# Isomorpfishm/SINGA

Hardware: AMD Instinct MI355X
Metric: protein-ligand graphs/sec GAN step (G+D fwd+bwd); scatter-TP kernel HBM GB/s (higher is better)
Workload: dtype f32

## Files before the change

### singa_amd/csrc/singa_hip.hip

```cpp
#include <hip/hip_runtime.h>
#include <hip/hip_ext.h>

#include <math.h>
#include <stdint.h>
#include <stdio.h>
#include <string.h>
#include <type_traits>

#include "../../include/singa_hip.h"
#include "../../include/singa_hip_lab.h"
#include "../../include/singa_hip_gen.h"
#include "../../include/singa_hip_force.h"
#include "so3_index.h"

namespace {

thread_local char g_err[256] = "ok";

int fail(int code, const char* msg) {
    snprintf(g_err, sizeof(g_err), "%s", msg);
    return code;
}

int check_launch(const char* what) {
// ... 3207 lines not shown
    const int n0 = (int)(blockIdx.x / HV) * npb;
    const int n1 = n0 + npb < N ? n0 + npb : N;
    if (n0 >= n1) return;
    float w[L + 1][4][4];
#pragma unroll
    for (int l = 0; l <= L; ++l)
#pragma unroll
        for (int t = 0; t < 4; ++t)
#pragma unroll
            for (int j = 0; j < 4; ++j) w[l][t][j] = W[l * w_l + (cc + t) * w_c + (4 * g + j) * w_u];
    float4 bc = make_float4(0.f, 0.f, 0.f, 0.f);
    if (bias) bc = *reinterpret_cast<const float4*>(bias + cc);
    for (int nb = n0; nb < n1; nb += 16) {
        const int na = nb + i < n1 ? nb + i : n1 - 1;
        const float* arow = small + (long long)na * K * 16 + 4 * g;
        float4 a = *reinterpret_cast<const float4*>(arow);
#pragma unroll
        for (int k = 0; k < K; ++k) {
            float4 an = a;
            if (k + 1 < K) an = *reinterpret_cast<const float4*>(arow + (k + 1) * 16);
            int l = 0;
            while ((l + 1) * (l + 1) <= k) ++l;
            const float av[4] = {a.x, a.y, a.z, a.w};
            floatx4 acc[4];
#pragma unroll
            for (int t = 0; t < 4; ++t) {
                const float b0 = k == 0 ? (t == 0 ? bc.x : (t == 1 ? bc.y : (t == 2 ? bc.z : bc.w))) : 0.f;
                acc[t] = floatx4{b0, b0, b0, b0};
            }
#pragma unroll
            for (int j = 0; j < 4; ++j)
#pragma unroll
                for (int t = 0; t < 4; ++t) acc[t] = __builtin_amdgcn_mfma_f32_16x16x4f32(av[j], w[l][t][j], acc[t], 0, 0, 0);
#pragma unroll
            for (int r = 0; r < 4; ++r) {
                const int n = nb + 4 * g + r;
                if (act && n < n1)
                    *reinterpret_cast<float4*>(big + ((long long)n * K + k) * C + cc) = make_float4(acc[0][r], acc[1][r], acc[2][r], acc[3][r]);
            }
            a = an;
        }
    }
}

template <int L>
struct SkinnyChunk {
    static constexpr int K = (L + 1) * (L + 1);
    static constexpr int D = L == 2 ? 3 : (L == 4 ? 5 : 7);
};

template <int L, int C>
__global__ void __launch_bounds__(SkinnyCfg<C>::BLOCK) so3_skinny_reduce_mfma_kernel(const float* __restrict__ small, const float* __restrict__ big,
                                                                     float* __restrict__ part, int N, int npb, int out_cu,
                                                                     int bias_row) {
    constexpr int K = (L + 1) * (L + 1), HV = SkinnyCfg<C>::HALVES, BL = SkinnyCfg<C>::BLOCK, D = SkinnyChunk<L>::D, NCH = K / D;
    static_assert(NCH * D == K, "chunking");
    const int lane = threadIdx.x & 63, i = lane & 15, g = lane >> 4;
    const int c0 = ((int)(blockIdx.x % HV) * (BL / 64) + (int)(threadIdx.x >> 6)) * 64 + 4 * i;
    const bool act = c0 + 3 < C;
    const int cc = act ? c0 : C - 4;
    const int n0 = (int)(blockIdx.x / HV) * npb;
    const int n1 = n0 + npb < N ? n0 + npb : N;
    floatx4 acc[L + 1][4];
#pragma unroll
    for (int l = 0; l <= L; ++l)
#pragma unroll
        for (int t = 0; t < 4; ++t) acc[l][t] = floatx4{0.f, 0.f, 0.f, 0.f};
    float4 accb = make_float4(0.f, 0.f, 0.f, 0.f);
    if (n0 < n1) {
        float4 bcur[D], bnxt[D];
        float acur[D], anxt[D];
        auto load = [&](float4* b, float* a, int q, int ch) {
            const int n = q + g;
            const bool ok = n < n1;
            const long long nn = ok ? n : n1 - 1;
#pragma unroll
            for (int d = 0; d < D; ++d) {
                const int k = ch * D + d;
                b[d] = *reinterpret_cast<const float4*>(big + (nn * K + k) * C + cc);
                const float v = small[(nn * K + k) * 16 + i];
                a[d] = ok ? v : 0.f;
            }
        };
        load(bnxt, anxt, n0, 0);
        for (int q = n0; q < n1; q += 4) {
#pragma unroll
            for (int ch = 0; ch < NCH; ++ch) {
#pragma unroll
                for (int d = 0; d < D; ++d) bcur[d] = bnxt[d], acur[d] = anxt[d];
                if (ch + 1 < NCH) load(bnxt, anxt, q, ch + 1);
                else load(bnxt, anxt, q + 4 < n1 ? q + 4 : q, 0);
#pragma unroll
                for (int d = 0; d < D; ++d) {
                    const int k = ch * D + d;
                    int l = 0;
                    while ((l + 1) * (l + 1) <= k) ++l;
                    const float bv[4] = {bcur[d].x, bcur[d].y, bcur[d].z, bcur[d].w};
#pragma unroll
                    for (int t = 0; t < 4; ++t) acc[l][t] = __builtin_amdgcn_mfma_f32_16x16x4f32(acur[d], bv[t], acc[l][t], 0, 0, 0);
                    if (k == 0 && q + g < n1) {
                        accb.x += bv[0]; accb.y += bv[1]; accb.z += bv[2]; accb.w += bv[3];
                    }
                }
            }
        }
    }
    constexpr int WSZ_ = (L + 1) * 16 * C;
    float* p = part + (long long)(blockIdx.x / HV) * (WSZ_ + (bias_row ? C : 0));
    if (bias_row) {
        accb.x += __shfl_xor(accb.x, 16, 64); accb.y += __shfl_xor(accb.y, 16, 64); accb.z += __shfl_xor(accb.z, 16, 64); accb.w += __shfl_xor(accb.w, 16, 64);
        accb.x += __shfl_xor(accb.x, 32, 64); accb.y += __shfl_xor(accb.y, 32, 64); accb.z += __shfl_xor(accb.z, 32, 64); accb.w += __shfl_xor(accb.w, 32, 64);
    }
    if (!act) return;
#pragma unroll
    for (int l = 0; l <= L; ++l) {
        if (out_cu) {
#pragma unroll
            for (int t = 0; t < 4; ++t)
                *reinterpret_cast<float4*>(p + ((long long)l * C + cc + t) * 16 + 4 * g) = make_float4(acc[l][t][0], acc[l][t][1], acc[l][t][2], acc[l][t][3]);
        } else {
#pragma unroll
            for (int r = 0; r < 4; ++r)
                *reinterpret_cast<float4*>(p + ((long long)l * 16 + 4 * g + r) * C + cc) = make_float4(acc[l][0][r], acc[l][1][r], acc[l][2][r], acc[l][3][r]);
        }
    }
    if (bias_row && g == 0) *reinterpret_cast<float4*>(p + WSZ_ + cc) = accb;
}

static inline int so3_skinny_npb(int N, int target_blocks) {
    int npb = (N + target_blocks - 1) / target_blocks;
    return npb < 8 ? 8 : npb;
}

template <int C>
static int so3_skinny_reduce_runs(int lmax) {
    static int cached[8] = {0};
    if (lmax < 0 || lmax > 7) return 512;
    if (cached[lmax]) return cached[lmax];
    int per_cu = 0, cus = 256;
    hipError_t e = hipErrorInvalidValue;
    constexpr int BL = SkinnyCfg<C>::BLOCK;
    if (lmax == 2) e = hipOccupancyMaxActiveBlocksPerMultiprocessor(&per_cu, so3_skinny_reduce_kernel<2, C>, BL, 0);
    if (lmax == 4) e = hipOccupancyMaxActiveBlocksPerMultiprocessor(&per_cu, so3_skinny_reduce_kernel<4, C>, BL, 0);
    if (lmax == 6) e = hipOccupancyMaxActiveBlocksPerMultiprocessor(&per_cu, so3_skinny_reduce_kernel<6, C>, BL, 0);
    if (e != hipSuccess || per_cu < 1) per_cu = 2;
    int dev = 0;
    hipDeviceProp_t prop;
    if (hipGetDevice(&dev) == hipSuccess && hipGetDeviceProperties(&prop, dev) == hipSuccess && prop.multiProcessorCount > 0)
        cus = prop.multiProcessorCount;
    cached[lmax] = per_cu * cus / SkinnyCfg<C>::HALVES;
    return cached[lmax];
}
static inline bool so3_skinny_channels_ok(int C) { return C == 512 || C == 112; }

__device__ __forceinline__ float group16_sum(float v) {
    v += __shfl_xor(v, 1, 64);
    v += __shfl_xor(v, 2, 64);
    v += __shfl_xor(v, 4, 64);
    v += __shfl_xor(v, 8, 64);
    return v;
}
__host__ __device__ constexpr int deg_of_c(int k) {
    int l = 0;
    while ((l + 1) * (l + 1) <= k) ++l;
    return l;
}
__host__ __device__ constexpr float bal_of_c(int k, int L) { return 1.0f / (float)((2 * deg_of_c(k) + 1) * (L + 1)); }

template <int L>
__global__ void __launch_bounds__(64) rmsnorm_fwd4_kernel(const float* __restrict__ x, const float* __restrict__ weight,
                                                          const float* __restrict__ bias, float* __restrict__ y, int N, float eps) {
    constexpr int C = 16, K = (L + 1) * (L + 1), KC = K * C;
    const int lane = threadIdx.x, q = lane >> 4, c = lane & 15;
    float w[L + 1];
#pragma unroll
    for (int l = 0; l <= L; ++l) w[l] = weight[l * C + c];
    const float bc = bias[c];
    for (int n0 = 4 * (int)blockIdx.x; n0 < N; n0 += 4 * (int)gridDim.x) {
        const int n = n0 + q;
        const bool ok = n < N;
        const float* xi = x + (long long)(ok ? n : N - 1) * KC + c;
        float v[K];
#pragma clang loop unroll(full)
        for (int k = 0; k < K; ++k) v[k] = xi[k * C];
        v[0] -= group16_sum(v[0]) * (1.0f / C);
        float ss = 0.f;
#pragma clang loop unroll(full)
        for (int k = 0; k < K; ++k) ss = fmaf(v[k] * v[k], bal_of_c(k, L), ss);
        const float r = rsqrtf(group16_sum(ss) * (1.0f / C) + eps);
        if (ok) {
            float* yo = y + (long long)n * KC + c;
#pragma clang loop unroll(full)
            for (int k = 0; k < K; ++k) {
                const float rw = r * w[deg_of_c(k)];
                yo[k * C] = k == 0 ? fmaf(v[k], rw, bc) : v[k] * rw;
            }
        }
    }
}

template <int L, bool ADD>
__global__ void __launch_bounds__(64) rmsnorm_bwd4_kernel(const float* __restrict__ x, const float* __restrict__ weight,
                                                          const float* __restrict__ gy, const float* __restrict__ g_add,
                                                          float* __restrict__ gx, float* __restrict__ gw_part,
                                                          float* __restrict__ gb_part, int N, float eps) {
    constexpr int C = 16, K = (L + 1) * (L + 1), KC = K * C;
    const int lane = threadIdx.x, q = lane >> 4, c = lane & 15;
    float w[L + 1], gwp[L + 1];
#pragma unroll
    for (int l = 0; l <= L; ++l) { w[l] = weight[l * C + c]; gwp[l] = 0.f; }
    float gbp = 0.f;
    for (int n0 = 4 * (int)blockIdx.x; n0 < N; n0 += 4 * (int)gridDim.x) {
        const int n = n0 + q;
        const bool ok = n < N;
        const long long base = (long long)(ok ? n : N - 1) * KC + c;
        float v[K], g[K], ga[ADD ? K : 1];
#pragma clang loop unroll(full)
        for (int k = 0; k < K; ++k) {
            v[k] = x[base + k * C];
            g[k] = gy[base + k * C];
            if constexpr (ADD) ga[k] = g_add[base + k * C];
        }
        const float live = ok ? 1.f : 0.f;
        v[0] -= group16_sum(v[0]) * (1.0f / C);
        float ss = 0.f, gl[L + 1];
#pragma unroll
        for (int l = 0; l <= L; ++l) gl[l] = 0.f;
#pragma clang loop unroll(full)
        for (int k = 0; k < K; ++k) {
            ss = fmaf(v[k] * v[k], bal_of_c(k, L), ss);
            gl[deg_of_c(k)] = fmaf(g[k], v[k], gl[deg_of_c(k)]);
        }
        float S = 0.f;
#pragma unroll
        for (int l = 0; l <= L; ++l) S = fmaf(gl[l], w[l], S);
        gbp = fmaf(g[0], live, gbp);
        const float r = rsqrtf(group16_sum(ss) * (1.0f / C) + eps);
        S = group16_sum(S);
        const float r3s = r * r * r * S * (1.0f / C);
#pragma unroll
        for (int l = 0; l <= L; ++l) gwp[l] = fmaf(gl[l] * live, r, gwp[l]);
        float* go = gx + base;
        float d0 = fmaf(r * w[0], g[0], -r3s * bal_of_c(0, L) * v[0]);
        d0 -= group16_sum(d0) * (1.0f / C);
        if (ok) {
            go[0] = ADD ? d0 + ga[0] : d0;
#pragma clang loop unroll(full)
            for (int k = 1; k < K; ++k) {
                const float d = fmaf(r * w[deg_of_c(k)], g[k], -r3s * bal_of_c(k, L) * v[k]);
                go[k * C] = ADD ? d + ga[k] : d;
            }
        }
    }
#pragma unroll
    for (int l = 0; l <= L; ++l) {
        gwp[l] += __shfl_xor(gwp[l], 16, 64);
        gwp[l] += __shfl_xor(gwp[l], 32, 64);
    }
    gbp += __shfl_xor(gbp, 16, 64);
    gbp += __shfl_xor(gbp, 32, 64);
    if (lane < C) {
        float* wp = gw_part + (long long)blockIdx.x * (L + 1) * C;
#pragma unroll
        for (int l = 0; l <= L; ++l) wp[l * C + c] = gwp[l];
        gb_part[(long long)blockIdx.x * C + c] = gbp;
    }
}


__global__ void __launch_bounds__(64) knn_edge_attr_kernel(const float* __restrict__ len, const int* __restrict__ ptr, long long n_real,
                                                           const float* __restrict__ offset, float coeff, float* __restrict__ out, int N) {
    const int g = threadIdx.x;
    const float off = offset[g];
    SINGA_XCD_NODE_LOOP(i, N) {
        const int beg = ptr[i], end = ptr[i + 1];
        float deg = 0.f;
        int e = beg;
        for (; e + 3 < end; e += 4) {
            float d[4], v[4];
#pragma unroll
            for (int q = 0; q < 4; ++q) d[q] = (e + q < n_real ? len[e + q] : 0.f) - off;
#pragma unroll
            for (int q = 0; q < 4; ++q) {
                const float sq = d[q] * d[q];
                v[q] = e + q < n_real ? expf(coeff * sq) : 0.f;
            }
#pragma unroll
            for (int q = 0; q < 4; ++q) {
                out[((long long)(e + q) + i) * 64 + g] = -v[q];
                deg += v[q];
            }
        }
        for (; e < end; ++e) {
            const float dd = (e < n_real ? len[e] : 0.f) - off;
            const float sq = dd * dd;
            const float v = e < n_real ? expf(coeff * sq) : 0.f;
            out[((long long)e + i) * 64 + g] = -v;
            deg += v;
        }
        out[((long long)end + i) * 64 + g] = deg;
    }
}

struct GemmProb {
    const float* A;
    const float* B;
    float* C;
    const float* bias;
    const float* mask;
    const float* addend;
    float* asum;
    long long asum_stride;
    long long lda, ldb, ldc, a_gld, b_gld, c_gld, c_split;
    int I, J, R, a_group, b_group, c_group, tiles_j, tile_begin, relu;
};
struct GemmBatch {
    GemmProb p[SINGA_GEMM_MAX];
    int n, tiles_total, splits, tj_total;
    long long r_chunk;
};

#ifndef SINGA_GEMM_PIPE
#define SINGA_GEMM_PIPE 1
#endif
#if SINGA_GEMM_PIPE
#define SINGA_GEMM_FENCE() do { if constexpr (CFG != 0 || !decltype(all_c)::value) __builtin_amdgcn_sched_barrier(0); } while (0)
#else
#define SINGA_GEMM_FENCE() __builtin_amdgcn_sched_barrier(0)
#endif
template <bool A_RC, bool B_RC, int CFG>
__global__ void __launch_bounds__(256, 2) gemm_f32_kernel(GemmBatch gb) {
    constexpr int BM = CFG == 2 ? 32 : (CFG == 3 ? 64 : 128), BN = CFG == 1 ? 32 : (CFG == 3 ? 64 : 128), BK = 32, PR = BK + 4;
    constexpr int MT = CFG == 0 ? 2 : 1, NT = CFG == 0 ? 2 : 1;
    constexpr int NA = BM / 32, NB = BN / 32;
    constexpr int LDA = BM + 4, LDB = BN + 4;
    constexpr int SZA = A_RC ? BM * PR : BK * LDA, SZB = B_RC ? BN * PR : BK * LDB;
    constexpr int PE = 32 * NT + 4;
    constexpr int SMEM = 2 * SZA + 2 * SZB > 4 * 32 * PE ? 2 * SZA + 2 * SZB : 4 * 32 * PE;
    __shared__ __attribute__((aligned(16))) float smem[SMEM];
    float* const As0 = smem;
    float* const Bs0 = smem + 2 * SZA;
    const int nblk = gb.tiles_total * gb.splits;
    const int per = (nblk + 7) >> 3;
    const int id = (int)(blockIdx.x & 7) * per + (int)(blockIdx.x >> 3);
    if (id >= nblk) return;
    const int split = id / gb.tiles_total;
    const int tile = id - split * gb.tiles_total;
    const int ti = gb.tj_total ? tile / gb.tj_total : 0, trem = gb.tj_total ? tile - ti * gb.tj_total : tile;
    int pi = 0;
#pragma unroll
    for (int q = 1; q < SINGA_GEMM_MAX; ++q)
        if (q < gb.n && trem >= gb.p[q].tile_begin) pi = q;
    const GemmProb& P = gb.p[pi];
    const int local = trem - P.tile_begin;
    const int i0 = (gb.tj_total ? ti : local / P.tiles_j) * BM, j0 = (gb.tj_total ? local : local % P.tiles_j) * BN;
    const long long r_begin = (long long)split * gb.r_chunk;
    const long long r_end = (r_begin + gb.r_chunk < P.R) ? r_begin + gb.r_chunk : P.R;
    const int tid = threadIdx.x, lane = tid & 63, wave = tid >> 6;
    const int wrow = CFG == 0 ? (wave >> 1) * 64 : (CFG == 1 ? wave * 32 : (CFG == 3 ? (wave >> 1) * 32 : 0));
    const int wcol = CFG == 0 ? (wave & 1) * 64 : (CFG == 1 ? 0 : (CFG == 3 ? (wave & 1) * 32 : wave * 32));
    const int l31 = lane & 31, half = lane >> 5;
    const int kq = tid & 7, rr = tid >> 3;

    const float* arow[NA];
    const float* brow[NB];
    if (A_RC) {
#pragma unroll
        for (int j = 0; j < NA; ++j) {
            const int i = i0 + rr + 32 * j;
            const long long off = P.a_group == (1 << 30) ? (long long)i * P.lda
                                                         : (long long)(i / P.a_group) * P.a_gld + (long long)(i % P.a_group) * P.lda;
            arow[j] = i < P.I ? P.A + off + 4 * kq : nullptr;
        }
    }
    if (B_RC) {
#pragma unroll
        for (int j = 0; j < NB; ++j) {
            const int jj = j0 + rr + 32 * j;
            brow[j] = jj < P.J ? P.B + (long long)jj * P.ldb + 4 * kq : nullptr;
        }
    }
    float4 ra0[NA], rb0[NB], ra1[NA], rb1[NB];
    const bool full = i0 + BM <= P.I && j0 + BN <= P.J && r_end > r_begin && (r_end - r_begin) % BK == 0;
    auto load_rc = [&](auto all_c, float4* reg, unsigned& mask, const float* const* rows, const float* dummy, int n, long long r0) {
        if constexpr (decltype(all_c)::value) {
#pragma unroll
            for (int j = 0; j < n; ++j) reg[j] = *reinterpret_cast<const float4*>(rows[j] + r0);
            mask = ~0u;
        } else {
            const bool in = r0 + 4 * kq < r_end;
            mask = 0;
#pragma unroll
            for (int j = 0; j < n; ++j) {
                const bool ok = in && rows[j] != nullptr;
                const float* src = ok ? rows[j] + r0 : dummy + r_begin;
                reg[j] = *reinterpret_cast<const float4*>(src);
                mask |= (ok ? 1u : 0u) << j;
            }
        }
    };
    auto load_oc = [&](auto all_c, float4* reg, unsigned& mask, const float* base, long long ld, int grp, long long gld, int o0,
                       int lim, int n, int width4, long long r0) {
        const int c4 = tid % width4, rq = tid / width4, rows = 256 / width4;
        const int i = o0 + 4 * c4;
        if constexpr (decltype(all_c)::value) {
            const float* b = base + (r0 + rq) * ld + i;
#pragma unroll
            for (int j = 0; j < n; ++j) reg[j] = *reinterpret_cast<const float4*>(b + (long long)(rows * j) * ld);
            mask = ~0u;
        } else {
            const int ic = i < lim ? i : o0;
            mask = 0;
#pragma unroll
            for (int j = 0; j < n; ++j) {
                const long long r = r0 + rq + rows * j;
                const bool ok = r < r_end && i < lim;
                const unsigned ru = (unsigned)(r < r_end ? r : r_begin), gq = ru / (unsigned)grp;
                const long long row = (long long)gq * gld + (long long)(ru - gq * (unsigned)grp) * ld;
                reg[j] = *reinterpret_cast<const float4*>(base + row + ic);
                mask |= (ok ? 1u : 0u) << j;
            }
        }
    };
    auto store_rc = [&](float* S, const float4* reg, unsigned mask, int n) {
#pragma unroll
        for (int j = 0; j < n; ++j)
            *reinterpret_cast<float4*>(S + (rr + 32 * j) * PR + 4 * kq) = (mask >> j) & 1u ? reg[j] : make_float4(0.f, 0.f, 0.f, 0.f);
    };
    auto store_oc = [&](float* S, const float4* reg, unsigned mask, int pitch, int n, int width4) {
        const int c4 = tid % width4, rq = tid / width4, rows = 256 / width4;
#pragma unroll
        for (int j = 0; j < n; ++j)
            *reinterpret_cast<float4*>(S + (rq + rows * j) * pitch + 4 * c4) = (mask >> j) & 1u ? reg[j] : make_float4(0.f, 0.f, 0.f, 0.f);
    };
    auto load_ab = [&](auto all_c, float4* ra, float4* rb, unsigned& ma, unsigned& mb, long long r0) __attribute__((always_inline)) {
        if (A_RC) load_rc(all_c, ra, ma, arow, P.A, NA, r0);
        else load_oc(all_c, ra, ma, P.A, P.lda, P.a_group, P.a_gld, i0, P.I, NA, BM / 4, r0);
        if (B_RC) load_rc(all_c, rb, mb, brow, P.B, NB, r0);
        else load_oc(all_c, rb, mb, P.B, P.ldb, P.b_group, P.b_gld, j0, P.J, NB, BN / 4, r0);
    };
    const bool do_asum = !A_RC && P.asum != nullptr && j0 == 0;
    const float asum_on = do_asum ? 1.f : 0.f;
    float4 asum4 = make_float4(0.f, 0.f, 0.f, 0.f);
    auto store_ab = [&](const float4* ra, const float4* rb, unsigned ma, unsigned mb, int buf) __attribute__((always_inline)) {
        if constexpr (!A_RC) {
#pragma unroll
            for (int j = 0; j < NA; ++j) {
                const float wj = ((ma >> j) & 1u) ? asum_on : 0.f;
                asum4.x = fmaf(wj, ra[j].x, asum4.x); asum4.y = fmaf(wj, ra[j].y, asum4.y);
                asum4.z = fmaf(wj, ra[j].z, asum4.z); asum4.w = fmaf(wj, ra[j].w, asum4.w);
            }
        }
        if (A_RC) store_rc(As0 + buf * SZA, ra, ma, NA);
        else store_oc(As0 + buf * SZA, ra, ma, LDA, NA, BM / 4);
        if (B_RC) store_rc(Bs0 + buf * SZB, rb, mb, NB);
        else store_oc(Bs0 + buf * SZB, rb, mb, LDB, NB, BN / 4);
    };
    const int ia = wrow + l31, jb = wcol + l31;
    auto frag = [&](const float* S, bool rc, int pitch, int col, int t, float (&f)[4]) __attribute__((always_inline)) {
        if (rc) {
            const float4 v = *reinterpret_cast<const float4*>(S + col * PR + 8 * t + 4 * half);
            f[0] = v.x; f[1] = v.y; f[2] = v.z; f[3] = v.w;
        } else {
#pragma unroll
            for (int q = 0; q < 4; ++q) f[q] = S[(8 * t + q + 4 * half) * pitch + col];
        }
    };

    floatx16 acc[MT][NT];
#pragma unroll
    for (int a = 0; a < MT; ++a)
#pragma unroll
        for (int b = 0; b < NT; ++b)
#pragma unroll
            for (int r = 0; r < 16; ++r) acc[a][b][r] = 0.f;

    unsigned blkv = 0;
#pragma unroll
    for (int a = 0; a < MT; ++a)
#pragma unroll
        for (int b = 0; b < NT; ++b)
            blkv |= ((i0 + wrow + 32 * a < P.I) && (j0 + wcol + 32 * b < P.J) ? 1u : 0u) << (a * NT + b);
    blkv = __builtin_amdgcn_readfirstlane(blkv);
    auto compute = [&](auto edge_c, int buf, int nt8) __attribute__((always_inline)) {
        const float* Sa = As0 + buf * SZA;
        const float* Sb = Bs0 + buf * SZB;
        float fa[2][MT][4], fb[2][NT][4];
#pragma unroll
        for (int a = 0; a < MT; ++a) frag(Sa, A_RC, LDA, ia + 32 * a, 0, fa[0][a]);
#pragma unroll
        for (int b = 0; b < NT; ++b) frag(Sb, B_RC, LDB, jb + 32 * b, 0, fb[0][b]);
#pragma unroll
        for (int t = 0; t < BK / 8; ++t) {
            if (t >= nt8) break;
            const int cur = t & 1;
            if (t + 1 < BK / 8) {
#pragma unroll
                for (int a = 0; a < MT; ++a) frag(Sa, A_RC, LDA, ia + 32 * a, t + 1, fa[cur ^ 1][a]);
#pragma unroll
                for (int b = 0; b < NT; ++b) frag(Sb, B_RC, LDB, jb + 32 * b, t + 1, fb[cur ^ 1][b]);
            }
#pragma unroll
            for (int q = 0; q < 4; ++q)
#pragma unroll
                for (int a = 0; a < MT; ++a)
#pragma unroll
                    for (int b = 0; b < NT; ++b) {
                        if constexpr (decltype(edge_c)::value) {
                            if ((blkv >> (a * NT + b)) & 1u)
                                acc[a][b] = __builtin_amdgcn_mfma_f32_32x32x2f32(fa[cur][a][q], fb[cur][b][q], acc[a][b], 0, 0, 0);
                        } else {
                            acc[a][b] = __builtin_amdgcn_mfma_f32_32x32x2f32(fa[cur][a][q], fb[cur][b][q], acc[a][b], 0, 0, 0);
                        }
                    }
        }
    };

    const long long nsteps = r_end > r_begin ? (r_end - r_begin + BK - 1) / BK : 0;
    const int last8 = nsteps > 0 ? (int)((r_end - r_begin - (nsteps - 1) * BK + 7) / 8) : 0;
    auto pipeline = [&](auto interior_c) __attribute__((always_inline)) {
#if SINGA_GEMM_PIPE
        if constexpr (CFG == 0 && decltype(interior_c)::value) {
            constexpr int DSR = (A_RC ? MT : 4 * MT) + (B_RC ? NT : 4 * NT);
            constexpr int MF = 0x008, VM = 0x020, DR = 0x100, DW = 0x200;
            __builtin_amdgcn_sched_group_barrier(DR, DSR, 0);
#pragma unroll
            for (int i = 0; i < 8; ++i) {
                __builtin_amdgcn_sched_group_barrier(MF, 2, 0);
                __builtin_amdgcn_sched_group_barrier(VM, 1, 0);
                if (i % 2 == 1) __builtin_amdgcn_sched_group_barrier(DR, DSR / 4, 0);
            }
#pragma unroll
            for (int g2 = 0; g2 < 2; ++g2)
#pragma unroll
                for (int i = 0; i < 4; ++i) {
                    __builtin_amdgcn_sched_group_barrier(MF, 4, 0);
                    __builtin_amdgcn_sched_group_barrier(DR, DSR / 4, 0);
                }
#pragma unroll
            for (int i = 0; i < 8; ++i) {
                __builtin_amdgcn_sched_group_barrier(MF, 2, 0);
                __builtin_amdgcn_sched_group_barrier(DW, 1, 0);
            }
        }
#endif
    };
    auto k_loop = [&](auto all_c) __attribute__((always_inline)) {
        constexpr std::integral_constant<bool, !decltype(all_c)::value> edge_c{};
        unsigned ma0 = 0, mb0 = 0, ma1 = 0, mb1 = 0;
        if (nsteps > 0) {
            load_ab(all_c, ra0, rb0, ma0, mb0, r_begin);
            if (nsteps > 1) load_ab(all_c, ra1, rb1, ma1, mb1, r_begin + BK);
            store_ab(ra0, rb0, ma0, mb0, 0);
        }
        __syncthreads();
        long long st = 0;
#if !defined(SINGA_GEMM_LAB_NOLOAD) && !defined(SINGA_GEMM_LAB_NOSYNC)
        if (nsteps > 3) __builtin_amdgcn_s_waitcnt(0x0F70);
        for (; st + 3 < nsteps; st += 2) {
            load_ab(all_c, ra0, rb0, ma0, mb0, r_begin + (st + 2) * BK);
            SINGA_GEMM_FENCE();
            compute(edge_c, 0, 4);
            SINGA_GEMM_FENCE();
            store_ab(ra1, rb1, ma1, mb1, 1);
            pipeline(all_c);
            __syncthreads();
            load_ab(all_c, ra1, rb1, ma1, mb1, r_begin + (st + 3) * BK);
            SINGA_GEMM_FENCE();
            compute(edge_c, 1, 4);
            SINGA_GEMM_FENCE();
            store_ab(ra0, rb0, ma0, mb0, 0);
            pipeline(all_c);
            __syncthreads();
        }
#endif
        for (; st < nsteps; st += 2) {
#if defined(SINGA_GEMM_LAB_NOLOAD) || defined(SINGA_GEMM_LAB_NOSYNC)
            compute(edge_c, 0, 4);
#ifndef SINGA_GEMM_LAB_NOSYNC
            if (st + 1 < nsteps) store_ab(ra1, rb1, ma1, mb1, 1);
            __syncthreads();
#endif
            if (st + 1 >= nsteps) break;
            compute(edge_c, 1, 4);
#ifndef SINGA_GEMM_LAB_NOSYNC
            if (st + 2 < nsteps) store_ab(ra0, rb0, ma0, mb0, 0);
            __syncthreads();
#endif
#else
            if (st + 2 < nsteps) load_ab(all_c, ra0, rb0, ma0, mb0, r_begin + (st + 2) * BK);
            compute(edge_c, 0, st + 1 == nsteps ? last8 : 4);
            if (st + 1 < nsteps) store_ab(ra1, rb1, ma1, mb1, 1);
            __syncthreads();
            if (st + 1 >= nsteps) break;
            if (st + 3 < nsteps) load_ab(all_c, ra1, rb1, ma1, mb1, r_begin + (st + 3) * BK);
            compute(edge_c, 1, st + 2 == nsteps ? last8 : 4);
            if (st + 2 < nsteps) store_ab(ra0, rb0, ma0, mb0, 0);
            __syncthreads();
#endif
        }
    };
    if (full && P.a_group == (1 << 30) && P.b_group == (1 << 30)) k_loop(std::true_type{});
    else k_loop(std::false_type{});
    if (!A_RC && do_asum) {
        constexpr int W4 = BM / 4, RG = 256 / W4;
        float* red = smem;
        *reinterpret_cast<float4*>(red + (tid / W4) * BM + 4 * (tid % W4)) = asum4;
        __syncthreads();
        if (tid < BM) {
            float t = 0.f;
#pragma unroll
            for (int g2 = 0; g2 < RG; ++g2) t += red[g2 * BM + tid];
            if (i0 + tid < P.I) P.asum[(long long)split * P.asum_stride + i0 + tid] = t;
        }
        __syncthreads();
    }
    float* Cb = P.C + (long long)split * P.c_split;
    float* stage = smem + wave * (32 * PE);
    constexpr int C4 = 8 * NT;
    constexpr int ROWS_PER_PASS = 64 / C4, PASSES = 32 / ROWS_PER_PASS;
    const int c4 = lane % C4, rsub = lane / C4;
    const int jcol = j0 + wcol + 4 * c4;
    float4 bias4 = make_float4(0.f, 0.f, 0.f, 0.f);
    if (P.bias && jcol < P.J) bias4 = *reinterpret_cast<const float4*>(P.bias + jcol);
#pragma unroll
    for (int a = 0; a < MT; ++a) {
        __builtin_amdgcn_wave_barrier();
#pragma unroll
        for (int b = 0; b < NT; ++b)
#pragma unroll
            for (int q = 0; q < 16; ++q) stage[((q & 3) + 8 * (q >> 2) + 4 * half) * PE + 32 * b + l31] = acc[a][b][q];
        __builtin_amdgcn_wave_barrier();
#pragma unroll
        for (int ps = 0; ps < PASSES; ++ps) {
            const int rloc = rsub + ROWS_PER_PASS * ps;
            const int i = i0 + wrow + 32 * a + rloc;
            float4 v = *reinterpret_cast<const float4*>(stage + rloc * PE + 4 * c4);
            if (i < P.I && jcol < P.J) {
                v.x += bias4.x; v.y += bias4.y; v.z += bias4.z; v.w += bias4.w;
                const long long row = P.c_group == (1 << 30) ? (long long)i * P.ldc
                                                             : (long long)(i / P.c_group) * P.c_gld + (long long)(i % P.c_group) * P.ldc;
                if (P.addend) {
                    const float4 ad = *reinterpret_cast<const float4*>(P.addend + row + jcol);
                    v.x += ad.x; v.y += ad.y; v.z += ad.z; v.w += ad.w;
                }
                if (P.relu) { v.x = fmaxf(v.x, 0.f); v.y = fmaxf(v.y, 0.f); v.z = fmaxf(v.z, 0.f); v.w = fmaxf(v.w, 0.f); }
                if (P.mask) {
                    const float4 m = *reinterpret_cast<const float4*>(P.mask + row + jcol);
                    v.x = m.x > 0.f ? v.x : 0.f; v.y = m.y > 0.f ? v.y : 0.f; v.z = m.z > 0.f ? v.z : 0.f; v.w = m.w > 0.f ? v.w : 0.f;
                }
                *reinterpret_cast<float4*>(Cb + row + jcol) = v;
            }
        }
    }
}

struct CGemmProb {
    const float* A;
    const float* B;
    float* C;
    long long lda, ldb, ldc, a_im, b_im, c_im, c_split;
    int I, J, R, tiles_j, tile_begin;
    float sigma;
};
struct CGemmBatch {
    CGemmProb p[SINGA_CGEMM_MAX];
    int n, tiles_total, splits, tj_total;
    long long r_chunk;
};

#ifndef SINGA_CGEMM_PIPE
#define SINGA_CGEMM_PIPE 1
#endif
#if SINGA_CGEMM_PIPE
#define SINGA_CGEMM_FENCE() do { if constexpr (!decltype(all_c)::value) __builtin_amdgcn_sched_barrier(0); } while (0)
#else
#define SINGA_CGEMM_FENCE() __builtin_amdgcn_sched_barrier(0)
#endif
template <bool A_RC, bool B_RC>
__global__ void __launch_bounds__(256, 2) cgemm3m_f32_kernel(CGemmBatch gb) {
    constexpr int BM = 128, BN = 64, BK = 16, PR = BK + 4, LDA = BM + 4, LDB = BN + 4;
    constexpr int NA = 4, NB = 2;
    constexpr int SZA1 = A_RC ? BM * PR : BK * LDA, SZB1 = B_RC ? BN * PR : BK * LDB;
    constexpr int SZA = 2 * SZA1, SZB = 2 * SZB1;
    constexpr int PE = 64 + 4;
    constexpr int SMEM = 2 * SZA + 2 * SZB > 4 * 32 * PE ? 2 * SZA + 2 * SZB : 4 * 32 * PE;
    __shared__ __attribute__((aligned(16))) float smem[SMEM];
    float* const As0 = smem;
    float* const Bs0 = smem + 2 * SZA;
    const int nblk = gb.tiles_total * gb.splits;
    const int per = (nblk + 7) >> 3;
    const int id = (int)(blockIdx.x & 7) * per + (int)(blockIdx.x >> 3);
    if (id >= nblk) return;
    const int split = id / gb.tiles_total;
    const int tile = id - split * gb.tiles_total;
    const int ti = gb.tj_total ? tile / gb.tj_total : 0, trem = gb.tj_total ? tile - ti * gb.tj_total : tile;
    int pi = 0;
#pragma unroll
    for (int q = 1; q < SINGA_CGEMM_MAX; ++q)
        if (q < gb.n && trem >= gb.p[q].tile_begin) pi = q;
    const CGemmProb& P = gb.p[pi];
    const int local = trem - P.tile_begin;
    const int i0 = (gb.tj_total ? ti : local / P.tiles_j) * BM, j0 = (gb.tj_total ? local : local % P.tiles_j) * BN;
    const long long r_begin = (long long)split * gb.r_chunk;
    const long long r_end = (r_begin + gb.r_chunk < P.R) ? r_begin + gb.r_chunk : P.R;
    const int tid = threadIdx.x, lane = tid & 63, wave = tid >> 6;
    const int wrow = (wave >> 1) * 64, wcol = (wave & 1) * 32;
    const int l31 = lane & 31, half = lane >> 5;
    const float sigma = P.sigma;

    const int kq = tid & 3, pt = (tid >> 2) & 1, rr = tid >> 3;
    const float* arow[NA];
    const float* brow[NB];
    if (A_RC) {
#pragma unroll
        for (int j = 0; j < NA; ++j) {
            const int i = i0 + rr + 32 * j;
            arow[j] = i < P.I ? P.A + (long long)i * P.lda + (long long)pt * P.a_im + 4 * kq : nullptr;
        }
    }
    if (B_RC) {
#pragma unroll
        for (int j = 0; j < NB; ++j) {
            const int jj = j0 + rr + 32 * j;
            brow[j] = jj < P.J ? P.B + (long long)jj * P.ldb + (long long)pt * P.b_im + 4 * kq : nullptr;
        }
    }
    float4 ra0[NA], rb0[NB], ra1[NA], rb1[NB];
    const bool full = i0 + BM <= P.I && j0 + BN <= P.J && r_end > r_begin && (r_end - r_begin) % BK == 0;
    auto load_rc = [&](auto all_c, float4* reg, unsigned& mask, const float* const* rows, const float* dummy, int n, long long r0) {
        if constexpr (decltype(all_c)::value) {
#pragma unroll
            for (int j = 0; j < n; ++j) reg[j] = *reinterpret_cast<const float4*>(rows[j] + r0);
            mask = ~0u;
        } else {
            const bool in = r0 + 4 * kq < r_end;
            mask = 0;
#pragma unroll
            for (int j = 0; j < n; ++j) {
                const bool ok = in && rows[j] != nullptr;
                const float* src = ok ? rows[j] + r0 : dummy + r_begin;
                reg[j] = *reinterpret_cast<const float4*>(src);
                mask |= (ok ? 1u : 0u) << j;
            }
        }
    };
    auto load_oc = [&](auto all_c, float4* reg, unsigned& mask, const float* base, long long ld, long long im, int o0, int lim, int n,
                       int width4, long long r0) {
        const int c4 = tid % width4, rq = tid / width4, rows = 256 / width4;
        const int i = o0 + 4 * c4;
        if constexpr (decltype(all_c)::value) {
            const float* b = base + (r0 + rq) * ld + i;
#pragma unroll
            for (int j = 0; j < n; ++j) {
                const int part = j / (n / 2), ps = j % (n / 2);
                reg[j] = *reinterpret_cast<const float4*>(b + (long long)part * im + (long long)(rows * ps) * ld);
            }
            mask = ~0u;
        } else {
            const int ic = i < lim ? i : o0;
            mask = 0;
#pragma unroll
            for (int j = 0; j < n; ++j) {
                const int part = j / (n / 2), ps = j % (n / 2);
                const long long r = r0 + rq + rows * ps;
                const bool ok = r < r_end && i < lim;
                const long long rc = r < r_end ? r : r_begin;
                reg[j] = *reinterpret_cast<const float4*>(base + rc * ld + (long long)part * im + ic);
                mask |= (ok ? 1u : 0u) << j;
            }
        }
    };
    auto store_rc = [&](float* S, int sz1, const float4* reg, unsigned mask, int n) {
#pragma unroll
        for (int j = 0; j < n; ++j)
            *reinterpret_cast<float4*>(S + pt * sz1 + (rr + 32 * j) * PR + 4 * kq) =
                (mask >> j) & 1u ? reg[j] : make_float4(0.f, 0.f, 0.f, 0.f);
    };
    auto store_oc = [&](float* S, int sz1, const float4* reg, unsigned mask, int pitch, int n, int width4) {
        const int c4 = tid % width4, rq = tid / width4, rows = 256 / width4;
#pragma unroll
        for (int j = 0; j < n; ++j) {
            const int part = j / (n / 2), ps = j % (n / 2);
            *reinterpret_cast<float4*>(S + part * sz1 + (rq + rows * ps) * pitch + 4 * c4) =
                (mask >> j) & 1u ? reg[j] : make_float4(0.f, 0.f, 0.f, 0.f);
        }
    };
    auto load_ab = [&](auto all_c, float4* ra, float4* rb, unsigned& ma, unsigned& mb, long long r0) __attribute__((always_inline)) {
        if (A_RC) load_rc(all_c, ra, ma, arow, P.A, NA, r0);
        else load_oc(all_c, ra, ma, P.A, P.lda, P.a_im, i0, P.I, NA, BM / 4, r0);
        if (B_RC) load_rc(all_c, rb, mb, brow, P.B, NB, r0);
        else load_oc(all_c, rb, mb, P.B, P.ldb, P.b_im, j0, P.J, NB, BN / 4, r0);
    };
    auto store_ab = [&](const float4* ra, const float4* rb, unsigned ma, unsigned mb, int buf) __attribute__((always_inline)) {
        if (A_RC) store_rc(As0 + buf * SZA, SZA1, ra, ma, NA);
        else store_oc(As0 + buf * SZA, SZA1, ra, ma, LDA, NA, BM / 4);
        if (B_RC) store_rc(Bs0 + buf * SZB, SZB1, rb, mb, NB);
        else store_oc(Bs0 + buf * SZB, SZB1, rb, mb, LDB, NB, BN / 4);
    };
    const int ia = wrow + l31, jb = wcol + l31;
    auto frag = [&](const float* S, bool rc, int pitch, int col, int t, float (&f)[4]) __attribute__((always_inline)) {
        if (rc) {
            const float4 v = *reinterpret_cast<const float4*>(S + col * PR + 8 * t + 4 * half);
            f[0] = v.x; f[1] = v.y; f[2] = v.z; f[3] = v.w;
        } else {
#pragma unroll
            for (int q = 0; q < 4; ++q) f[q] = S[(8 * t + q + 4 * half) * pitch + col];
        }
    };
    floatx16 acc1[2], acc2[2], acc3[2];
#pragma unroll
    for (int a = 0; a < 2; ++a)
#pragma unroll
        for (int r = 0; r < 16; ++r) acc1[a][r] = acc2[a][r] = acc3[a][r] = 0.f;
    const bool row1 = __builtin_amdgcn_readfirstlane((int)(i0 + wrow + 32 < P.I)) != 0;
    const bool colv = __builtin_amdgcn_readfirstlane((int)(j0 + wcol < P.J)) != 0;
    auto compute = [&](auto all_c, int buf) __attribute__((always_inline)) {
        if constexpr (!decltype(all_c)::value) {
            if (!colv) return;
        }
        const float* Sa = As0 + buf * SZA;
        const float* Sb = Bs0 + buf * SZB;
#pragma unroll
        for (int t = 0; t < BK / 8; ++t) {
            float ar[2][4], ai[2][4], br[4], bi[4];
#pragma unroll
            for (int a = 0; a < 2; ++a) {
                frag(Sa, A_RC, LDA, ia + 32 * a, t, ar[a]);
                frag(Sa + SZA1, A_RC, LDA, ia + 32 * a, t, ai[a]);
            }
            frag(Sb, B_RC, LDB, jb, t, br);
            frag(Sb + SZB1, B_RC, LDB, jb, t, bi);
#pragma unroll
            for (int q = 0; q < 4; ++q) {
                const float ds = sigma * bi[q];
                const float b2 = ds - br[q], b3 = ds + br[q];
                acc1[0] = __builtin_amdgcn_mfma_f32_32x32x2f32(ar[0][q] + ai[0][q], br[q], acc1[0], 0, 0, 0);
                acc2[0] = __builtin_amdgcn_mfma_f32_32x32x2f32(ar[0][q], b2, acc2[0], 0, 0, 0);
                acc3[0] = __builtin_amdgcn_mfma_f32_32x32x2f32(ai[0][q], b3, acc3[0], 0, 0, 0);
                if (decltype(all_c)::value || row1) {
                    acc1[1] = __builtin_amdgcn_mfma_f32_32x32x2f32(ar[1][q] + ai[1][q], br[q], acc1[1], 0, 0, 0);
                    acc2[1] = __builtin_amdgcn_mfma_f32_32x32x2f32(ar[1][q], b2, acc2[1], 0, 0, 0);
                    acc3[1] = __builtin_amdgcn_mfma_f32_32x32x2f32(ai[1][q], b3, acc3[1], 0, 0, 0);
                }
            }
        }
    };
    const long long nsteps = r_end > r_begin ? (r_end - r_begin + BK - 1) / BK : 0;
    auto pipeline = [&](auto interior_c) __attribute__((always_inline)) {
#if SINGA_CGEMM_PIPE
        if constexpr (decltype(interior_c)::value) {
            constexpr int DSR = (A_RC ? 4 : 16) + (B_RC ? 2 : 8);
            constexpr int MF = 0x008, VM = 0x020, DR = 0x100, DW = 0x200;
            __builtin_amdgcn_sched_group_barrier(DR, DSR, 0);
#pragma unroll
            for (int i = 0; i < 6; ++i) {
                __builtin_amdgcn_sched_group_barrier(MF, 4, 0);
                __builtin_amdgcn_sched_group_barrier(VM, 1, 0);
                __builtin_amdgcn_sched_group_barrier(DR, (DSR + 5) / 6, 0);
            }
#pragma unroll
            for (int i = 0; i < 6; ++i) {
                __builtin_amdgcn_sched_group_barrier(MF, 4, 0);
                __builtin_amdgcn_sched_group_barrier(DW, 1, 0);
            }
        }
#endif
    };
    auto k_loop = [&](auto all_c) __attribute__((always_inline)) {
        unsigned ma0 = 0, mb0 = 0, ma1 = 0, mb1 = 0;
        if (nsteps > 0) {
            load_ab(all_c, ra0, rb0, ma0, mb0, r_begin);
            if (nsteps > 1) load_ab(all_c, ra1, rb1, ma1, mb1, r_begin + BK);
            store_ab(ra0, rb0, ma0, mb0, 0);
        }
        __syncthreads();
        long long st = 0;
        if (nsteps > 3) __builtin_amdgcn_s_waitcnt(0x0F70);
        for (; st + 3 < nsteps; st += 2) {
            load_ab(all_c, ra0, rb0, ma0, mb0, r_begin + (st + 2) * BK);
            SINGA_CGEMM_FENCE();
            compute(all_c, 0);
            SINGA_CGEMM_FENCE();
            store_ab(ra1, rb1, ma1, mb1, 1);
            pipeline(all_c);
            __syncthreads();
            load_ab(all_c, ra1, rb1, ma1, mb1, r_begin + (st + 3) * BK);
            SINGA_CGEMM_FENCE();
            compute(all_c, 1);
            SINGA_CGEMM_FENCE();
            store_ab(ra0, rb0, ma0, mb0, 0);
            pipeline(all_c);
            __syncthreads();
        }
        for (; st < nsteps; st += 2) {
            if (st + 2 < nsteps) load_ab(all_c, ra0, rb0, ma0, mb0, r_begin + (st + 2) * BK);
            compute(all_c, 0);
            if (st + 1 < nsteps) store_ab(ra1, rb1, ma1, mb1, 1);
            __syncthreads();
            if (st + 1 >= nsteps) break;
            if (st + 3 < nsteps) load_ab(all_c, ra1, rb1, ma1, mb1, r_begin + (st + 3) * BK);
            compute(all_c, 1);
            if (st + 2 < nsteps) store_ab(ra0, rb0, ma0, mb0, 0);
            __syncthreads();
        }
    };
    if (full) k_loop(std::true_type{});
    else k_loop(std::false_type{});
    float* Cb = P.C + (long long)split * P.c_split;
    float* stage = smem + wave * (32 * PE);
    const int c4 = lane & 15, rsub = lane >> 4;
    const int part = c4 >> 3, jcol = j0 + wcol + 4 * (c4 & 7);
#pragma unroll
    for (int a = 0; a < 2; ++a) {
        __builtin_amdgcn_wave_barrier();
#pragma unroll
        for (int q = 0; q < 16; ++q) {
            const int rw = (q & 3) + 8 * (q >> 2) + 4 * half;
            stage[rw * PE + l31] = acc1[a][q] - acc3[a][q];
            stage[rw * PE + 32 + l31] = acc1[a][q] + acc2[a][q];
        }
        __builtin_amdgcn_wave_barrier();
#pragma unroll
        for (int ps = 0; ps < 8; ++ps) {
            const int rloc = rsub + 4 * ps;
            const int i = i0 + wrow + 32 * a + rloc;
            const float4 v = *reinterpret_cast<const float4*>(stage + rloc * PE + 4 * c4);
            if (i < P.I && jcol < P.J)
                *reinterpret_cast<float4*>(Cb + (long long)i * P.ldc + (long long)part * P.c_im + jcol) = v;
        }
    }
}

__global__ void __launch_bounds__(256) block_weight_fwd_kernel(const float* __restrict__ w, float* __restrict__ out, int h, int k) {
    const long long t = (long long)blockIdx.x * blockDim.x + threadIdx.x;
    if (t >= 4LL * h * k) return;
    const int i = (int)(t / (2 * k)), j = (int)(t - (long long)i * 2 * k);
    float v;
    if (i < h) v = j < k ? w[(long long)i * k + j] : -w[(long long)(h + i) * k + (j - k)];
    else v = j < k ? w[(long long)i * k + j] : w[(long long)(i - h) * k + (j - k)];
    out[t] = v;
}
__global__ void __launch_bounds__(256) block_weight_bwd_kernel(const float* __restrict__ G, float* __restrict__ gw, int h, int k, int accumulate) {
    const long long t = (long long)blockIdx.x * blockDim.x + threadIdx.x;
    if (t >= 2LL * h * k) return;
    const int i = (int)(t / k), j = (int)(t - (long long)i * k);
    float v;
    if (i < h) v = G[(long long)i * 2 * k + j] + G[(long long)(h + i) * 2 * k + k + j];
    else v = G[(long long)i * 2 * k + j] - G[(long long)(i - h) * 2 * k + k + j];
    gw[t] = accumulate ? gw[t] + v : v;
}

__global__ void __launch_bounds__(256) rowdot32_fwd_kernel(const float* __restrict__ x, const float* __restrict__ b, float* __restrict__ out,
                                                           long long M, float scale) {
    const long long row = ((long long)blockIdx.x * 256 + threadIdx.x) >> 3;
    const int q = threadIdx.x & 7;
    float s = 0.f;
    if (row < M) {
        const float4 xv = *reinterpret_cast<const float4*>(x + row * 32 + 4 * q);
        const float4 bv = *reinterpret_cast<const float4*>(b + 4 * q);
        s = xv.x * bv.x + xv.y * bv.y + xv.z * bv.z + xv.w * bv.w;
    }
    s += __shfl_xor(s, 1, 64);
    s += __shfl_xor(s, 2, 64);
    s += __shfl_xor(s, 4, 64);
    if (row < M && q == 0) out[row] = s * scale;
}
constexpr int ROWDOT_ROWS = 256;
__global__ void __launch_bounds__(256) rowdot32_bwd_kernel(const float* __restrict__ g, const float* __restrict__ x, const float* __restrict__ b,
                                                           float* __restrict__ gx, float* __restrict__ part, long long M, float scale) {
    __shared__ float red[32][33];
    const int q = threadIdx.x & 7, r = threadIdx.x >> 3;
    const float4 bv = *reinterpret_cast<const float4*>(b + 4 * q);
    float4 acc = make_float4(0.f, 0.f, 0.f, 0.f);
    const long long r0 = (long long)blockIdx.x * ROWDOT_ROWS;
    for (int p = 0; p < ROWDOT_ROWS / 32; ++p) {
        const long long row = r0 + p * 32 + r;
        if (row < M) {
            const float gs = g[row] * scale;
            const float4 xv = *reinterpret_cast<const float4*>(x + row * 32 + 4 * q);
            *reinterpret_cast<float4*>(gx + row * 32 + 4 * q) = make_float4(gs * bv.x, gs * bv.y, gs * bv.z, gs * bv.w);
            acc.x = fmaf(gs, xv.x, acc.x); acc.y = fmaf(gs, xv.y, acc.y); acc.z = fmaf(gs, xv.z, acc.z); acc.w = fmaf(gs, xv.w, acc.w);
        }
    }
    red[r][4 * q] = acc.x, red[r][4 * q + 1] = acc.y, red[r][4 * q + 2] = acc.z, red[r][4 * q + 3] = acc.w;
    __syncthreads();
    if (threadIdx.x < 32) {
        float s = 0.f;
        for (int i = 0; i < 32; ++i) s += red[i][threadIdx.x];
        part[(long long)blockIdx.x * 32 + threadIdx.x] = s;
    }
}

#ifndef SINGA_EMUL
constexpr int LAP_FSI_PB = 16, LAP_FSI_ELLW = 32, LAP_FSI_DEG = 24, LAP_FSI_MAXIT = 40;
constexpr int LAP_FSI_PER_LD = 3 * LAP_FSI_PB + LAP_FSI_ELLW + LAP_FSI_ELLW / 2;
constexpr int LAP_WORK_PER_LD = 3 + 4 * 9 + LAP_FSI_PER_LD;
template <int NW, int KV>
__device__ __forceinline__ bool lap_fsi(const double* __restrict__ A, int ld, int n, int sl, const int* perm, const int* cbeg,
                                        const int* cend, int* ell_n, int* flag, double* Xl, double* sc, double* wk, int m, int tid,
                                        int lane, int wave) {
    constexpr int PB = LAP_FSI_PB, W = LAP_FSI_ELLW;
    double* Yg = wk;
    double* Wg = Yg + (long long)ld * PB;
    double* Ng = Wg + (long long)ld * PB;
    double* ell_v = Ng + (long long)ld * PB;
    int* ell_i = reinterpret_cast<int*>(ell_v + (long long)ld * W);
    double* H = sc;
    double* Q = sc + 256;
    double* part = sc + 512;
    double* theta = sc + 1024;
    double* resn = theta + 16;
    double* misc = resn + 16;
    const int total = n * PB;
    (void)sl;
    if (tid == 0) flag[1] = 0;
    __syncthreads();
    for (int s0 = wave; s0 < n; s0 += NW) {
        const int lo = cbeg[s0], hi = cend[s0];
        const double* row = A + (long long)perm[s0] * ld;
        int cnt = 0;
        for (int t0 = lo; t0 <= hi; t0 += 64) {
            const int t = t0 + lane;
            const double v = t <= hi ? row[perm[t]] : 0.0;
            const bool nz = v != 0.0;
            const unsigned long long mask = __ballot(nz);
            const int at = cnt + __popcll(mask & ((1ull << lane) - 1ull));
            if (nz && at < W) {
                ell_i[(long long)s0 * W + at] = t;
                ell_v[(long long)s0 * W + at] = v;
            }
            cnt += __popcll(mask);
        }
        if (lane == 0) {
            ell_n[s0] = cnt < W ? cnt : W;
            if (cnt > W) flag[1] = 1;
        }
    }
    __syncthreads();
    if (flag[1]) return false;
    for (int idx = tid; idx < total; idx += 1024) {
        const int r = idx >> 4, j = idx & 15;
        unsigned h = (unsigned)(perm[r] * 2654435761u) ^ (unsigned)((j + 11) * 40503u * 2246822519u);
        h ^= h >> 15; h *= 2246822519u; h ^= h >> 13; h *= 3266489917u; h ^= h >> 16;
        Xl[idx] = (double)(h & 0xFFFFFF) / 8388608.0 - 1.0;
    }
    __syncthreads();
    auto lx = [&](int idx) -> double {
        const int r = idx >> 4, j = idx & 15;
        const int cnt = ell_n[r];
        const double* ev = ell_v + (long long)r * W;
        const int* ei = ell_i + (long long)r * W;
        double acc = 0.0;
        for (int e = 0; e < cnt; ++e) acc += ev[e] * Xl[ei[e] * PB + j];
        return acc;
    };
    auto gram = [&](const double* B) {
        if (tid < 512) {
            const int p = tid & 255, ch = tid >> 8, a = p >> 4, b = p & 15;
            double acc = 0.0;
            for (int r = ch; r < n; r += 2) acc += Xl[r * PB + a] * B[r * PB + b];
            part[ch * 256 + p] = acc;
        }
        __syncthreads();
        if (tid < 256) Q[tid] = part[tid] + part[256 + tid];
        __syncthreads();
        if (tid < 256) H[tid] = 0.5 * (Q[tid] + Q[(tid & 15) * 16 + (tid >> 4)]);
        __syncthreads();
    };
    auto orthonormalise = [&]() -> bool {
        for (int pass = 0; pass < 2; ++pass) {
            gram(Xl);
            if (tid == 0) {
                misc[0] = 0.0;
                double tr = 0.0;
                for (int j = 0; j < PB; ++j) tr += H[j * 16 + j];
                for (int j = 0; j < PB; ++j) {
                    double d = H[j * 16 + j];
                    for (int k = 0; k < j; ++k) d -= Q[k * 16 + j] * Q[k * 16 + j];
                    if (!(d > 1e-26 * tr)) { misc[0] = 1.0; d = 1.0; }
                    const double rj = sqrt(d);
                    Q[j * 16 + j] = rj;
                    for (int i = j + 1; i < PB; ++i) {
                        double v = H[j * 16 + i];
                        for (int k = 0; k < j; ++k) v -= Q[k * 16 + j] * Q[k * 16 + i];
                        Q[j * 16 + i] = v / rj;
                    }
                }
            }
            __syncthreads();
            if (misc[0] != 0.0) return false;
            if (tid < n) {
                double* xr = Xl + tid * PB;
#pragma unroll 1
                for (int j = 0; j < PB; ++j) {
                    double v = xr[j];
#pragma unroll 1
                    for (int i = 0; i < j; ++i) v -= xr[i] * Q[i * 16 + j];
                    xr[j] = v / Q[j * 16 + j];
                }
            }
            __syncthreads();
        }
        return true;
    };
    auto ritz = [&]() {
        for (int idx = tid; idx < total; idx += 1024) Wg[idx] = lx(idx);
        __syncthreads();
        gram(Wg);
        if (tid < 256) Q[tid] = (tid >> 4) == (tid & 15) ? 1.0 : 0.0;
        __syncthreads();
        for (int sweep = 0; sweep < 10; ++sweep) {
            if (tid == 0) {
                double off = 0.0, dg = 0.0;
                for (int i = 0; i < PB; ++i)
                    for (int j = 0; j < PB; ++j) (i == j ? dg : off) += H[i * 16 + j] * H[i * 16 + j];
                misc[1] = off <= 1e-30 * (dg + 1e-300) ? 1.0 : 0.0;
            }
            __syncthreads();
            const bool done = misc[1] != 0.0;
            __syncthreads();
            if (done) break;
            for (int st = 0; st < 15; ++st) {
                const int pr = tid >> 3, sub = tid & 7;
                const int p = pr == 0 ? 15 : (st + pr) % 15, q = pr == 0 ? st : (st + 15 - pr) % 15;
                double c = 1.0, sn = 0.0;
                if (tid < 64) {
                    const double hpp = H[p * 16 + p], hqq = H[q * 16 + q], hpq = H[p * 16 + q];
                    if (fabs(hpq) > 1e-300) {
                        const double tau = (hqq - hpp) / (2.0 * hpq);
                        const double t = (tau >= 0.0 ? 1.0 : -1.0) / (fabs(tau) + sqrt(1.0 + tau * tau));
                        c = 1.0 / sqrt(1.0 + t * t);
                        sn = t * c;
                    }
                }
                __syncthreads();
                if (tid < 64) {
#pragma unroll
                    for (int h2 = 0; h2 < 2; ++h2) {
                        const int i = sub + 8 * h2;
                        const double aip = H[i * 16 + p], aiq = H[i * 16 + q];
                        H[i * 16 + p] = c * aip - sn * aiq;
                        H[i * 16 + q] = sn * aip + c * aiq;
                        const double qip = Q[i * 16 + p], qiq = Q[i * 16 + q];
                        Q[i * 16 + p] = c * qip - sn * qiq;
                        Q[i * 16 + q] = sn * qip + c * qiq;
                    }
                }
                __syncthreads();
                if (tid < 64) {
#pragma unroll
                    for (int h2 = 0; h2 < 2; ++h2) {
                        const int i = sub + 8 * h2;
                        const double api = H[p * 16 + i], aqi = H[q * 16 + i];
                        H[p * 16 + i] = c * api - sn * aqi;
                        H[q * 16 + i] = sn * api + c * aqi;
                    }
                }
                __syncthreads();
            }
        }
        if (tid == 0) {
            int ord[PB];
            for (int j = 0; j < PB; ++j) ord[j] = j;
            for (int a = 1; a < PB; ++a) {
                const int oa = ord[a];
                int b = a;
                while (b > 0 && H[ord[b - 1] * 16 + ord[b - 1]] > H[oa * 16 + oa]) { ord[b] = ord[b - 1]; --b; }
                ord[b] = oa;
            }
            for (int j = 0; j < PB; ++j) {
                theta[j] = H[ord[j] * 16 + ord[j]];
                for (int i = 0; i < PB; ++i) part[i * 16 + j] = Q[i * 16 + ord[j]];
            }
        }
        __syncthreads();
        if (tid < n) {
            for (int which = 0; which < 2; ++which) {
                double* rowp = which == 0 ? Xl + tid * PB : Wg + tid * PB;
                double x[PB];
#pragma unroll
                for (int i = 0; i < PB; ++i) x[i] = rowp[i];
#pragma unroll 1
                for (int j = 0; j < PB; ++j) {
                    double xs = 0.0;
#pragma unroll
                    for (int i = 0; i < PB; ++i) xs += x[i] * part[i * 16 + j];
                    rowp[j] = xs;
                }
            }
        }
        __syncthreads();
        {
            const int j = tid & 15, ch = tid >> 4;
            const double th = theta[j];
            double acc = 0.0;
            for (int r = ch; r < n; r += 64) {
                const double d = Wg[r * PB + j] - th * Xl[r * PB + j];
                acc += d * d;
            }
            acc += __shfl_xor(acc, 16, 64);
            acc += __shfl_xor(acc, 32, 64);
            __syncthreads();
            if (lane < 16) part[wave * 16 + lane] = acc;
            __syncthreads();
            if (tid < PB) {
                double t = 0.0;
                for (int w2 = 0; w2 < NW; ++w2) t += part[w2 * 16 + tid];
                resn[tid] = sqrt(t);
            }
            __syncthreads();
        }
    };
    if (!orthonormalise()) return false;
    bool ok = false;
    for (int it = 0; it < LAP_FSI_MAXIT; ++it) {
        ritz();
        double worst = 0.0;
        for (int j = 0; j < m; ++j) worst = fmax(worst, resn[j]);
        if (worst <= 2e-10) { ok = true; break; }
        const double a0 = theta[0], b = 2.0 + 1e-9;
        const double a = fmax(theta[PB - 1], a0 + 1e-4);
        if (!(a < b - 1e-3)) break;
        const double e = 0.5 * (b - a), c = 0.5 * (b + a);
        double sigma = e / (a0 - c);
        const double sigma1 = sigma;
        for (int idx = tid; idx < total; idx += 1024) Ng[idx] = (lx(idx) - c * Xl[idx]) * (sigma1 / e);
        __syncthreads();
        for (int idx = tid; idx < total; idx += 1024) { Yg[idx] = Xl[idx]; Xl[idx] = Ng[idx]; }
        __syncthreads();
        for (int i = 2; i <= LAP_FSI_DEG; ++i) {
            const double sigma2 = 1.0 / (2.0 / sigma1 - sigma);
// ... 435 lines not shown
            const double b = bb[j];
            if (b == 0.0) continue;
            const double* v = A + (long long)perm[j] * ld;
            const int hi = cend[j];
            double s = 0.0;
            for (int r = j + 1 + lane; r <= hi; r += 64) s += v[perm[r]] * x[r];
#pragma unroll
            for (int o = 32; o > 0; o >>= 1) s += __shfl_xor(s, o, 64);
            s *= b;
            for (int r = j + 1 + lane; r <= hi; r += 64) x[r] -= s * v[perm[r]];
        }
    }
    }
    __syncthreads();
    float* o = out + (long long)first[g] * kout;
    for (int k = 1; k <= kout; ++k) {
        if (k >= m) {
            if (tid < n) o[(long long)tid * kout + k - 1] = 0.f;
            continue;
        }
        const double* x = Z + k * sl;
        double best = tid < n ? fabs(x[tid]) : -1.0;
        int bi = tid < n ? perm[tid] : (1 << 30), bp = tid;
#pragma unroll
        for (int oo = 32; oo > 0; oo >>= 1) {
            const double ob = __shfl_xor(best, oo, 64);
            const int oi = __shfl_xor(bi, oo, 64), op = __shfl_xor(bp, oo, 64);
            if (ob > best || (ob == best && oi < bi)) best = ob, bi = oi, bp = op;
        }
        __syncthreads();
        int* redi = reinterpret_cast<int*>(red + NW);
        if (lane == 0) red[wave] = best, redi[wave] = bi, redi[NW + wave] = bp;
        __syncthreads();
        best = red[0], bi = redi[0], bp = redi[NW];
        for (int w = 1; w < NW; ++w) {
            const double ob = red[w];
            const int oi = redi[w];
            if (ob > best || (ob == best && oi < bi)) best = ob, bi = oi, bp = redi[NW + w];
        }
        const double sg = x[bp] < 0.0 ? -1.0 : 1.0;
        if (tid < n) o[(long long)perm[tid] * kout + k - 1] = (float)(sg * x[tid]);
        __syncthreads();
    }
}
#endif

bool attn_pitch(int token_major, int heads, long long lq, long long lk, long long lv, const float* q, const float* k, const float* v,
                AttnPitch* out) {
    out->q = (int)(lq > 0 ? lq : heads * 32);
    out->k = (int)(lk > 0 ? lk : heads * 32);
    out->v = (int)(lv > 0 ? lv : heads * 64);
    if (!token_major) return lq <= 0 && lk <= 0 && lv <= 0;
    if (lq > (1 << 30) || lk > (1 << 30) || lv > (1 << 30)) return false;
    if (out->q % 4 || out->k % 4 || out->v % 4 || out->q < heads * 32 || out->k < heads * 32 || out->v < heads * 64) return false;
    return !(((uintptr_t)q & 15) || ((uintptr_t)k & 15) || ((uintptr_t)v & 15));
}

int grid_for(long long work, int cap = 256 * 32) {
    long long g = work < 1 ? 1 : work;
    return (int)(g > cap ? cap : g);
}
int kn_grid(long long N) {
    long long g = (N < 1 ? 1 : N);
    g = (g + 7) / 8 * 8;
    return (int)(g > (1 << 20) ? (1 << 20) : g);
}

bool pack(const singa_seg_t* s, int nseg, Segs* out) {
    if (!s || nseg < 1 || nseg > 3) return false;
    for (int i = 0; i < 3; ++i) {
        out->p[i] = i < nseg ? s[i].ptr : nullptr;
        out->ld[i] = i < nseg ? s[i].ld : 0;
        out->rows[i] = i < nseg ? s[i].rows : 0;
        if (i < nseg && !s[i].ptr) return false;
    }
    return true;
}

bool pack_mut(const singa_seg_mut_t* s, int nseg, SegsMut* out) {
    if (!s || nseg < 1 || nseg > 3) return false;
    for (int i = 0; i < 3; ++i) {
        out->p[i] = i < nseg ? s[i].ptr : nullptr;
        out->ld[i] = i < nseg ? s[i].ld : 0;
        out->rows[i] = i < nseg ? s[i].rows : 0;
        if (i < nseg && !s[i].ptr) return false;
    }
    return true;
}

#define SINGA_DISPATCH_L(lmax, mmax, ...)                                             \
    do {                                                                                \
        if ((mmax) != 2) return fail(SINGA_E_LMAX, "only mmax = 2 is built");           \
        switch (lmax) {                                                                 \
            case 2: { constexpr int L_ = 2; __VA_ARGS__; } break;                              \
            case 4: { constexpr int L_ = 4; __VA_ARGS__; } break;                              \
            case 6: { constexpr int L_ = 6; __VA_ARGS__; } break;                              \
            default: return fail(SINGA_E_LMAX, "lmax must be 2, 4 or 6");               \
        }                                                                               \
    } while (0)

template <int MAXC>
__global__ __launch_bounds__(256) void knn_graph_kernel(const float* __restrict__ pos, const int* __restrict__ batch,
                                                        const long long* __restrict__ ptr, int B, int N, int k,
                                                        long long* __restrict__ row, long long* __restrict__ col) {
    const int lane = threadIdx.x & 63;
    const int i = blockIdx.x * (blockDim.x >> 6) + (threadIdx.x >> 6);
    if (i >= N) return;
    const int g = batch[i];
    long long* ro = row + (long long)i * k;
    long long* co = col + (long long)i * k;
    if (g < 0 || g >= B) {
        for (int r = lane; r < k; r += 64) ro[r] = co[r] = -1;
        return;
    }
    const int lo = (int)ptr[g], hi = (int)ptr[g + 1];
    const float px = pos[3 * i], py = pos[3 * i + 1], pz = pos[3 * i + 2];
    const unsigned long long NONE = ~0ull;
    unsigned long long key[MAXC];
#pragma unroll
    for (int t = 0; t < MAXC; ++t) {
        const int c = lo + lane + 64 * t;
        key[t] = NONE;
        if (c < hi && c != i) {
            const float dx = __fsub_rn(px, pos[3 * c]), dy = __fsub_rn(py, pos[3 * c + 1]), dz = __fsub_rn(pz, pos[3 * c + 2]);
            const float d2 = __fadd_rn(__fadd_rn(__fmul_rn(dx, dx), __fmul_rn(dy, dy)), __fmul_rn(dz, dz));
            key[t] = ((unsigned long long)__float_as_uint(d2) << 32) | (unsigned)c;
        }
    }
    for (int r = 0; r < k; ++r) {
        unsigned long long best = key[0];
#pragma unroll
        for (int t = 1; t < MAXC; ++t) best = key[t] < best ? key[t] : best;
#pragma unroll
        for (int o = 32; o > 0; o >>= 1) {
            const unsigned blo = (unsigned)__shfl_xor((int)(unsigned)best, o, 64);
            const unsigned bhi = (unsigned)__shfl_xor((int)(unsigned)(best >> 32), o, 64);
            const unsigned long long other = ((unsigned long long)bhi << 32) | blo;
            best = other < best ? other : best;
        }
#pragma unroll
        for (int t = 0; t < MAXC; ++t)
            if (key[t] == best) key[t] = NONE;
        if (lane == 0) {
            const bool have = best != NONE;
            ro[r] = have ? (long long)i : -1;
            co[r] = have ? (long long)(unsigned)best : -1;
        }
    }
}

__global__ void calib_copy_kernel(const float* __restrict__ src, float* __restrict__ dst, long long n) {
    long long i = (long long)blockIdx.x * blockDim.x + threadIdx.x;
    long long stride = (long long)gridDim.x * blockDim.x;
    for (; i < n; i += stride) dst[i] = src[i];
}

template <int UNROLL>
__global__ void __launch_bounds__(256) calib_copy16_kernel(const float4* __restrict__ src, float4* __restrict__ dst, long long n4) {
    const long long chunk = 256LL * UNROLL;
    for (long long base = (long long)blockIdx.x * chunk; base < n4; base += (long long)gridDim.x * chunk) {
        float4 v[UNROLL];
#pragma unroll
        for (int u = 0; u < UNROLL; ++u) {
            const long long i = base + threadIdx.x + 256LL * u;
            if (i < n4) v[u] = src[i];
        }
#pragma unroll
        for (int u = 0; u < UNROLL; ++u) {
            const long long i = base + threadIdx.x + 256LL * u;
            if (i < n4) dst[i] = v[u];
        }
    }
}

}

extern "C" {

int singa_prof_enable(int on) {
    g_prof_on = on != 0;
    return SINGA_OK;
}

int singa_prof_stamps(unsigned long long* buf, int cap) {
    g_stamp_buf = buf;
    g_stamp_cap = buf ? cap : 0;
    if (buf) {
        g_prof_on = false;
        g_prof_n = 0;
    }
    return SINGA_OK;
}

int singa_prof_read_stamps(const unsigned long long* host_stamps, float* ms, int* tags, int* edges, int* nodes, int cap) {
    if (!host_stamps) return 0;
    int n = 0;
    double calib = (double)(host_stamps[1] - host_stamps[0]);
    for (int i = 1; i < g_prof_n && n < cap; ++i) {
        double ticks = (double)(host_stamps[2 * i + 1] - host_stamps[2 * i]) - calib;
        ms[n] = (float)(ticks * 1e-5);
        tags[n] = g_prof[i].tag;
        edges[n] = g_prof[i].E;
        nodes[n] = g_prof[i].N;
        ++n;
    }
    return n;
}

int singa_prof_reset(void) {
    g_prof_n = 0;
    return SINGA_OK;
}

int singa_prof_hint_edges(int E) {
    g_prof_edges_hint = E;
    return SINGA_OK;
}

int singa_prof_collect(float* ms, int* edges, int* nodes, int cap) {
    int n = 0;
    for (int i = 0; i < g_prof_n; ++i) {
        float t = 0.f;
        hipError_t e = hipEventElapsedTime(&t, g_prof[i].a, g_prof[i].b);
        if (e == hipSuccess && n < cap) {
            ms[n] = t;
            edges[n] = g_prof[i].E;
            nodes[n] = g_prof[i].N;
            ++n;
        }
        (void)hipEventDestroy(g_prof[i].a);
        (void)hipEventDestroy(g_prof[i].b);
    }
    g_prof_n = 0;
    return n;
}

int singa_prof_collect_tagged(float* ms, int* tags, int* edges, int* nodes, int cap) {
    int n = 0;
    for (int i = 0; i < g_prof_n; ++i) {
        float t = 0.f;
        hipError_t e = hipEventElapsedTime(&t, g_prof[i].a, g_prof[i].b);
        if (e == hipSuccess && n < cap) {
            ms[n] = t;
            tags[n] = g_prof[i].tag;
            edges[n] = g_prof[i].E;
            nodes[n] = g_prof[i].N;
            ++n;
        }
        (void)hipEventDestroy(g_prof[i].a);
        (void)hipEventDestroy(g_prof[i].b);
    }
    g_prof_n = 0;
    return n;
}

int singa_calib_copy(const float* src, float* dst, long long n, void* stream) {
    if (!src || !dst) return fail(SINGA_E_NULL, "calib_copy: null pointer");
    hipLaunchKernelGGL(calib_copy_kernel, dim3(256 * 8), dim3(256), 0, (hipStream_t)stream, src, dst, n);
    return check_launch("calib_copy");
}

int singa_knn_graph(const float* pos, const int32_t* batch, const long long* ptr, int B, int N, int k, int max_nodes, long long* row,
                    long long* col, void* stream) {
    if (!pos || !batch || !ptr || !row || !col) return fail(SINGA_E_NULL, "knn_graph: null pointer");
    if (B < 0 || N < 0 || k <= 0 || max_nodes < 0 || max_nodes > 2048) return fail(SINGA_E_SHAPE, "knn_graph: k > 0 and at most 2048 atoms per molecule");
    if (N == 0) return SINGA_OK;
    const dim3 grid((unsigned)((N + 3) / 4)), block(256);
    hipStream_t st = (hipStream_t)stream;
    if (max_nodes <= 512) hipLaunchKernelGGL(knn_graph_kernel<8>, grid, block, 0, st, pos, batch, ptr, B, N, k, row, col);
    else if (max_nodes <= 1024) hipLaunchKernelGGL(knn_graph_kernel<16>, grid, block, 0, st, pos, batch, ptr, B, N, k, row, col);
    else hipLaunchKernelGGL(knn_graph_kernel<32>, grid, block, 0, st, pos, batch, ptr, B, N, k, row, col);
    return check_launch("knn_graph");
}

int singa_knn_edge_attr(const float* len, const int32_t* ptr, long long n_real, const float* offset, float coeff, float* out, int N,
                        int G, void* stream) {
    if (!ptr || !offset || !out || (!len && n_real > 0)) return fail(SINGA_E_NULL, "knn_edge_attr: null pointer");
    if (G != 64) return fail(SINGA_E_SHAPE, "knn_edge_attr: 64 Gaussians (the shipped edge_channels)");
    if (N < 0 || n_real < 0) return fail(SINGA_E_SHAPE, "knn_edge_attr: negative size");
    if (N == 0) return SINGA_OK;
    hipLaunchKernelGGL(knn_edge_attr_kernel, dim3(kn_grid(N)), dim3(64), 0, (hipStream_t)stream, len, ptr, n_real, offset, coeff, out, N);
    return check_launch("knn_edge_attr");
}

int singa_calib_copy16(const float* src, float* dst, long long n, int blocks, int unroll, void* stream) {
    if (!src || !dst) return fail(SINGA_E_NULL, "calib_copy16: null pointer");
    if (n % 4 || ((uintptr_t)src | (uintptr_t)dst) % 16) return fail(SINGA_E_SHAPE, "calib_copy16: n % 4 == 0 and 16-byte aligned pointers");
    if (blocks < 1 || blocks > (1 << 20) || (unroll != 1 && unroll != 2 && unroll != 4 && unroll != 8))
        return fail(SINGA_E_SHAPE, "calib_copy16: blocks >= 1, unroll in {1, 2, 4, 8}");
    const float4* s4 = (const float4*)src;
    float4* d4 = (float4*)dst;
    hipStream_t st = (hipStream_t)stream;
    if (unroll == 1) hipLaunchKernelGGL(calib_copy16_kernel<1>, dim3(blocks), dim3(256), 0, st, s4, d4, n / 4);
    else if (unroll == 2) hipLaunchKernelGGL(calib_copy16_kernel<2>, dim3(blocks), dim3(256), 0, st, s4, d4, n / 4);
    else if (unroll == 4) hipLaunchKernelGGL(calib_copy16_kernel<4>, dim3(blocks), dim3(256), 0, st, s4, d4, n / 4);
    else hipLaunchKernelGGL(calib_copy16_kernel<8>, dim3(blocks), dim3(256), 0, st, s4, d4, n / 4);
    return check_launch("calib_copy16");
}

int singa_version(void) { return 100; }

const char* singa_last_error_string(void) { return g_err; }

int singa_init(const double* jd_flat, int lmax_max) {
    if (!jd_flat) return fail(SINGA_E_NULL, "singa_init: jd_flat is null");
    if (lmax_max < 0 || lmax_max > 11) return fail(SINGA_E_LMAX, "singa_init: lmax_max must be in [0, 11]");
    static float host[MAX_J];
    int n = j_off(lmax_max + 1);
    for (int i = 0; i < n; ++i) host[i] = (float)jd_flat[i];
    hipError_t e = hipMemcpyToSymbol(HIP_SYMBOL(g_J), host, n * sizeof(float), 0, hipMemcpyHostToDevice);
    if (e != hipSuccess) {
        snprintf(g_err, sizeof(g_err), "singa_init: %s", hipGetErrorString(e));
        return (int)e;
    }
    g_lmax_init = lmax_max;
    return SINGA_OK;
}

int singa_dims(int lmax, int mmax, int* kr, int* wsz, int* rad_rows) {
    SINGA_DISPATCH_L(lmax, mmax, {
        using I = SO3Idx<L_, 2>;
        if (kr) *kr = I::KR;
        if (wsz) *wsz = I::WSZ;
        if (rad_rows) *rad_rows = I::RAD_ROWS;
    });
    return SINGA_OK;
}

int singa_edge_frames(const float* vec, const float* rnd, float* rot, float* stats, int E, void* stream) {
    if (!vec || !rnd || !rot || !stats) return fail(SINGA_E_NULL, "edge_frames: null pointer");
    if (E <= 0) return SINGA_OK;
    hipLaunchKernelGGL(edge_frames_kernel, dim3((E + 255) / 256), dim3(256), 0, (hipStream_t)stream, vec, rnd, rot,
                       (int*)stats, E);
    return check_launch("edge_frames");
}

int singa_wigner_rows(const float* rot, float* wr, int E, int lmax, int mmax, void* stream) {
    if (!rot || !wr) return fail(SINGA_E_NULL, "wigner_rows: null pointer");
    if (g_lmax_init < lmax) return fail(SINGA_E_NOINIT, "wigner_rows: singa_init not called for this lmax");
    if (E <= 0) return SINGA_OK;
    SINGA_DISPATCH_L(lmax, mmax, {
        using I = SO3Idx<L_, 2>;
        long long total = (long long)E * I::KR;
        int blocks = (int)((total + 255) / 256);
        hipLaunchKernelGGL((wigner_rows_kernel<L_, 2>), dim3(blocks), dim3(256), 0, (hipStream_t)stream, rot, wr, E);
    });
    return check_launch("wigner_rows");
}

int singa_gather_rotate_fwd(const float* x_src, const float* x_dst, const int32_t* src, const int32_t* dst,
                            const float* wr, const float* rad, float* out, int E, int C, int lmax, int mmax,
                            void* stream) {
    if (!x_src || !x_dst || !src || !dst || !wr || !out) return fail(SINGA_E_NULL, "gather_rotate_fwd: null pointer");
    if (C != 16) return fail(SINGA_E_SHAPE, "gather_rotate: built for C = 16 sphere channels");
    if (E <= 0) return SINGA_OK;
    SINGA_DISPATCH_L(lmax, mmax, {
        if (rad)
            SINGA_LAUNCH(SINGA_PROF_K4_FWD, E, 0, (gather_rotate_kernel<L_, 2, 16, 0, true>), dim3(grid_for(E)), dim3(64),
                         (hipStream_t)stream, x_src, x_dst, src, dst, wr, rad, (const float*)nullptr, out, E);
        else
            SINGA_LAUNCH(SINGA_PROF_K4_FWD, E, 0, (gather_rotate_kernel<L_, 2, 16, 0, false>), dim3(grid_for(E)), dim3(64),
                         (hipStream_t)stream, x_src, x_dst, src, dst, wr, rad, (const float*)nullptr, out, E);
    });
    return check_launch("gather_rotate_fwd");
}

int singa_gather_rotate_bwd(const float* g_out, const float* x_src, const float* x_dst, const int32_t* src,
                            const int32_t* dst, const float* wr, const float* rad, const int32_t* row_ptr,
                            const int32_t* col_ptr, const int32_t* eperm, float* g_rad, float* gx_src, float* gx_dst,
                            int E, int Ns, int Nd, int C, int lmax, int mmax, void* stream) {
    if (!g_out || !x_src || !x_dst || !src || !dst || !wr || !row_ptr || !col_ptr || !eperm || !gx_src || !gx_dst)
        return fail(SINGA_E_NULL, "gather_rotate_bwd: null pointer");
    if (g_rad && !rad) return fail(SINGA_E_NULL, "gather_rotate_bwd: g_rad requested without rad");
    if (C != 16) return fail(SINGA_E_SHAPE, "gather_rotate: built for C = 16 sphere channels");
    SINGA_DISPATCH_L(lmax, mmax, {
        hipStream_t st = (hipStream_t)stream;
        if (g_rad && E > 0)
            SINGA_LAUNCH(SINGA_PROF_K4_BWD_RAD, E, 0, (gather_rotate_kernel<L_, 2, 16, 1, true>), dim3(grid_for(E)), dim3(64), st,
                         x_src, x_dst, src, dst, wr, rad, g_out, g_rad, E);
        if (Nd > 0) {
            if (rad)
                SINGA_LAUNCH(SINGA_PROF_K4_BWD_DST, E, Nd, (gather_rotate_bwd_node_kernel<L_, 2, 16, 0, true>),
                             dim3(grid_for((Nd + 15) / 16)), dim3(256), st, g_out, wr, rad, row_ptr, (const int*)nullptr, gx_dst, Nd);
            else
                SINGA_LAUNCH(SINGA_PROF_K4_BWD_DST, E, Nd, (gather_rotate_bwd_node_kernel<L_, 2, 16, 0, false>),
                             dim3(grid_for((Nd + 15) / 16)), dim3(256), st, g_out, wr, rad, row_ptr, (const int*)nullptr, gx_dst, Nd);
        }
        if (Ns > 0) {
            if (rad)
                SINGA_LAUNCH(SINGA_PROF_K4_BWD_SRC, E, Ns, (gather_rotate_bwd_node_kernel<L_, 2, 16, 1, true>),
                             dim3(grid_for((Ns + 15) / 16)), dim3(256), st, g_out, wr, rad, col_ptr, eperm, gx_src, Ns);
            else
                SINGA_LAUNCH(SINGA_PROF_K4_BWD_SRC, E, Ns, (gather_rotate_bwd_node_kernel<L_, 2, 16, 1, false>),
                             dim3(grid_for((Ns + 15) / 16)), dim3(256), st, g_out, wr, rad, col_ptr, eperm, gx_src, Ns);
        }
    });
    return check_launch("gather_rotate_bwd");
}

int singa_rotate_back_scatter_fwd(const singa_seg_t* msg, int nseg, const float* alpha, const float* wr,
                                  const int32_t* row_ptr, float* out, int Nd, int CH, int heads, int lmax, int mmax,
                                  int m0_only, float out_scale, void* stream) {
    Segs s;
    if (!pack(msg, nseg, &s) || !wr || !row_ptr || !out) return fail(SINGA_E_NULL, "rotate_back_scatter_fwd: null pointer");
    if (CH < 1 || CH > 128 || heads < 1 || CH % heads) return fail(SINGA_E_SHAPE, "rotate_back_scatter: CH must be <= 128 and divisible by heads");
    if (!m0_only && nseg != 3) return fail(SINGA_E_SHAPE, "rotate_back_scatter: full mode takes the 3 per-m segments");
    if (m0_only ? (CH != 16 || heads != 1) : (CH != 112 || heads != 7))
        return fail(SINGA_E_SHAPE, "rotate_back_scatter: built for 7 heads x 16 value channels (full) and 16 channels (m0_only)");
    if (Nd <= 0) return SINGA_OK;
    int bs = CH <= 64 ? 64 : 128;
    const int n_edges_hint = g_prof_edges_hint;
    SINGA_DISPATCH_L(lmax, mmax, {
        if (!m0_only && (s.rows[0] != L_ + 1 || s.rows[1] != 2 * L_ || s.rows[2] != 2 * (L_ - 1)))
            return fail(SINGA_E_SHAPE, "rotate_back_scatter: segment row counts must be L+1, 2L, 2(L-1)");
        if (m0_only)
            hipLaunchKernelGGL((rotate_back_scatter_kernel<L_, 2, true, 4, 16, 16>), dim3(grid_for(Nd, 1 << 20)), dim3(bs),
                               0, (hipStream_t)stream, s, alpha, wr, row_ptr, out, Nd, out_scale);
        else
            SINGA_LAUNCH(SINGA_PROF_K10_FWD, n_edges_hint, Nd,
                         (rotate_back_scatter_kernel<L_, 2, false, (L_ == 2 ? 4 : 0), 112, 16>), dim3(grid_for(Nd, 1 << 20)),
                         dim3(bs), (hipStream_t)stream, s, alpha, wr, row_ptr, out, Nd, out_scale);
    });
    return check_launch("rotate_back_scatter_fwd");
}

int singa_rotate_back_scatter_bwd(const float* g_out, const singa_seg_t* msg, const singa_seg_mut_t* g_msg, int nseg,
                                  const float* alpha, const float* wr, const int32_t* row_ptr, float* g_alpha_part,
                                  int Nd, int CH, int heads, int lmax, int mmax, int m0_only, float out_scale,
                                  void* stream) {
    Segs s;
    SegsMut gm;
    memset(&s, 0, sizeof(s));
    if (!g_out || !pack_mut(g_msg, nseg, &gm) || !wr || !row_ptr) return fail(SINGA_E_NULL, "rotate_back_scatter_bwd: null pointer");
    if (alpha && (!pack(msg, nseg, &s) || !g_alpha_part)) return fail(SINGA_E_NULL, "rotate_back_scatter_bwd: alpha given without msg / g_alpha_part");
    if (CH < 1 || CH > 128 || heads < 1 || CH % heads) return fail(SINGA_E_SHAPE, "rotate_back_scatter: CH must be <= 128 and divisible by heads");
    if (!m0_only && nseg != 3) return fail(SINGA_E_SHAPE, "rotate_back_scatter: full mode takes the 3 per-m segments");
    if (m0_only ? (CH != 16 || heads != 1) : (CH != 112 || heads != 7))
        return fail(SINGA_E_SHAPE, "rotate_back_scatter: built for 7 heads x 16 value channels (full) and 16 channels (m0_only)");
    if (Nd <= 0) return SINGA_OK;
    int bs = CH <= 64 ? 64 : 128;
    SINGA_DISPATCH_L(lmax, mmax, {
        if (!m0_only && (gm.rows[0] != L_ + 1 || gm.rows[1] != 2 * L_ || gm.rows[2] != 2 * (L_ - 1)))
            return fail(SINGA_E_SHAPE, "rotate_back_scatter: segment row counts must be L+1, 2L, 2(L-1)");
        if (m0_only)
            hipLaunchKernelGGL((rotate_back_scatter_bwd_kernel<L_, 2, true, 16, 16>), dim3(grid_for(Nd, 1 << 20)), dim3(bs), 0,
                               (hipStream_t)stream, g_out, s, gm, alpha, wr, row_ptr, g_alpha_part, Nd, out_scale);
        else
            SINGA_LAUNCH(SINGA_PROF_K10_BWD, g_prof_edges_hint, Nd, (rotate_back_scatter_bwd_kernel<L_, 2, false, 112, 16>),
                         dim3(grid_for(Nd, 1 << 20)), dim3(bs), (hipStream_t)stream, g_out, s, gm, alpha, wr, row_ptr,
                         g_alpha_part, Nd, out_scale);
    });
    return check_launch("rotate_back_scatter_bwd");
}

int singa_segment_softmax_fwd(const float* x, const int32_t* row_ptr, float* out, int N, int H, float eps,
                              int dense_segments, void* stream) {
    if (!x || !row_ptr || !out) return fail(SINGA_E_NULL, "segment_softmax_fwd: null pointer");
    if (N <= 0 || H <= 0) return SINGA_OK;
    if (H == 4 && dense_segments) {
        hipLaunchKernelGGL(segment_softmax4_fwd_kernel, dim3((N + 3) / 4), dim3(256), 0, (hipStream_t)stream, x, row_ptr, out, N,
                           eps);
        return check_launch("segment_softmax_fwd");
    }
    int blocks = (int)(((long long)N * H + 255) / 256);
    hipLaunchKernelGGL(segment_softmax_fwd_kernel, dim3(blocks), dim3(256), 0, (hipStream_t)stream, x, row_ptr, out, N,
                       H, eps);
    return check_launch("segment_softmax_fwd");
}

int singa_segment_softmax_bwd(const float* y, const float* gy, const int32_t* row_ptr, float* gx, int N, int H,
                              int dense_segments, void* stream) {
    if (!y || !gy || !row_ptr || !gx) return fail(SINGA_E_NULL, "segment_softmax_bwd: null pointer");
    if (N <= 0 || H <= 0) return SINGA_OK;
    if (H == 4 && dense_segments) {
        hipLaunchKernelGGL(segment_softmax4_bwd_kernel, dim3((N + 3) / 4), dim3(256), 0, (hipStream_t)stream, y, gy, row_ptr, gx, N);
        return check_launch("segment_softmax_bwd");
    }
    int blocks = (int)(((long long)N * H + 255) / 256);
    hipLaunchKernelGGL(segment_softmax_bwd_kernel, dim3(blocks), dim3(256), 0, (hipStream_t)stream, y, gy, row_ptr, gx,
                       N, H);
    return check_launch("segment_softmax_bwd");
}

int singa_segment_wsum_fwd(const float* w, const float* v, const int32_t* row_ptr, float* out, int N, int H, int F,
                           void* stream) {
    if (!w || !v || !row_ptr || !out) return fail(SINGA_E_NULL, "segment_wsum_fwd: null pointer");
    if (H * F > 1024 || H < 1 || F < 1) return fail(SINGA_E_SHAPE, "segment_wsum: H*F must be <= 1024");
    if (N <= 0) return SINGA_OK;
    int bs = ((H * F + 63) / 64) * 64;
    hipLaunchKernelGGL(segment_wsum_fwd_kernel, dim3(grid_for(N, 1 << 20)), dim3(bs), 0, (hipStream_t)stream, w, v,
                       row_ptr, out, N, H, F);
    return check_launch("segment_wsum_fwd");
}

int singa_segment_wsum_bwd(const float* g_out, const float* w, const float* v, const int32_t* row_ptr, float* gw,
                           float* gv, int N, int H, int F, void* stream) {
    if (!g_out || !w || !v || !row_ptr || !gw || !gv) return fail(SINGA_E_NULL, "segment_wsum_bwd: null pointer");
    if (H * F > 1024 || H < 1 || F < 1 || F > 64 || (F & (F - 1))) return fail(SINGA_E_SHAPE, "segment_wsum_bwd: F must be a power of two <= 64");
    if (N <= 0) return SINGA_OK;
    int bs = ((H * F + 63) / 64) * 64;
    hipLaunchKernelGGL(segment_wsum_bwd_kernel, dim3(grid_for(N, 1 << 20)), dim3(bs), 0, (hipStream_t)stream, g_out, w,
                       v, row_ptr, gw, gv, N, H, F);
    return check_launch("segment_wsum_bwd");
}

#define SINGA_DISPATCH_S2(kin, ch, nseg, ...)                                                            \
    do {                                                                                                 \
        if ((nseg) == 3 && (ch) == 128) {                                                                \
            constexpr int C_ = 128; constexpr bool EDGE_ = true;                                         \
            switch (kin) {                                                                               \
                case 9: { constexpr int KIN_ = 9; __VA_ARGS__; } break;                                  \
                case 19: { constexpr int KIN_ = 19; __VA_ARGS__; } break;                                \
                case 29: { constexpr int KIN_ = 29; __VA_ARGS__; } break;                                \
                default: return fail(SINGA_E_SHAPE, "s2act(edge): KIN must be 9, 19 or 29");             \
            }                                                                                            \
        } else if ((nseg) == 1 && (ch) == 512) {                                                         \
            constexpr int C_ = 512; constexpr bool EDGE_ = false;                                        \
            switch (kin) {                                                                               \
                case 9: { constexpr int KIN_ = 9; __VA_ARGS__; } break;                                  \
                case 25: { constexpr int KIN_ = 25; __VA_ARGS__; } break;                                \
                case 49: { constexpr int KIN_ = 49; __VA_ARGS__; } break;                                \
                default: return fail(SINGA_E_SHAPE, "s2act(node): KIN must be 9, 25 or 49");             \
            }                                                                                            \
        } else {                                                                                         \
            return fail(SINGA_E_SHAPE, "s2act: built for (3 segments, C = 128) and (1 segment, C = 512)"); \
        }                                                                                                \
    } while (0)

int singa_s2act_fwd(const singa_seg_t* x, int nseg, const float* gate, int64_t ldg, const float* to_grid,
                    const float* from_grid, float* out, int E, int C, int KIN, int G, void* stream) {
    Segs s;
    if (!pack(x, nseg, &s) || !gate || !to_grid || !from_grid || !out) return fail(SINGA_E_NULL, "s2act_fwd: null pointer");
    if (s.rows[0] + s.rows[1] + s.rows[2] != KIN) return fail(SINGA_E_SHAPE, "s2act: segment rows must sum to KIN");
    if (E <= 0) return SINGA_OK;
    long long EC = (long long)E * C;
    int blocks = (int)((EC + 255) / 256);
    if (nseg == 3 && (s.rows[0] != (KIN + 1) / 5 + 1 || s.rows[1] != 2 * ((KIN + 1) / 5)))
        return fail(SINGA_E_SHAPE, "s2act(edge): segment rows must be L+1, 2L, 2(L-1)");
    SINGA_DISPATCH_S2(KIN, C, nseg, hipLaunchKernelGGL((s2act_fwd_kernel<KIN_, C_, EDGE_>), dim3(blocks), dim3(256), 0,
                                                       (hipStream_t)stream, s, gate, (long long)ldg, to_grid, from_grid,
                                                       out, EC, G));
    return check_launch("s2act_fwd");
}

int singa_s2act_bwd(const singa_seg_t* x, int nseg, const float* gate, int64_t ldg, const float* to_grid,
                    const float* from_grid, const float* g_out, float* gx, float* g_gate, int E, int C, int KIN,
                    int G, void* stream) {
    Segs s;
    if (!pack(x, nseg, &s) || !gate || !to_grid || !from_grid || !g_out || !gx || !g_gate)
        return fail(SINGA_E_NULL, "s2act_bwd: null pointer");
    if (s.rows[0] + s.rows[1] + s.rows[2] != KIN) return fail(SINGA_E_SHAPE, "s2act: segment rows must sum to KIN");
    if (E <= 0) return SINGA_OK;
    long long EC = (long long)E * C;
    int blocks = (int)((EC + 255) / 256);
    if (nseg == 3 && (s.rows[0] != (KIN + 1) / 5 + 1 || s.rows[1] != 2 * ((KIN + 1) / 5)))
        return fail(SINGA_E_SHAPE, "s2act(edge): segment rows must be L+1, 2L, 2(L-1)");
    SINGA_DISPATCH_S2(KIN, C, nseg, hipLaunchKernelGGL((s2act_bwd_kernel<KIN_, C_, EDGE_>), dim3(blocks), dim3(256), 0,
                                                       (hipStream_t)stream, s, gate, (long long)ldg, to_grid, from_grid,
                                                       g_out, gx, g_gate, EC, G));
    return check_launch("s2act_bwd");
}

int singa_edge_logits_fwd(const float* qp, const float* wk, const float* hk, const float* cterm, const int32_t* row_ptr,
                          const int32_t* col, float* qk, int N, int H, int D, float scale, void* stream) {
    if (!qp || !wk || !hk || !cterm || !row_ptr || !col || !qk) return fail(SINGA_E_NULL, "edge_logits_fwd: null pointer");
    if (H != 4 || D != 32) return fail(SINGA_E_SHAPE, "edge_logits: built for H = 4 heads, D = 32 key channels per head");
    if (N <= 0) return SINGA_OK;
    hipLaunchKernelGGL((edge_logits_fwd_kernel<32, 4>), dim3(kn_grid(N)), dim3(64), 0, (hipStream_t)stream, qp, wk,
                       hk, cterm, row_ptr, col, qk, N, scale);
    return check_launch("edge_logits_fwd");
}

int singa_edge_logits_bwd(const float* g, const float* qp, const float* wk, const float* hk, const int32_t* row_ptr,
                          const int32_t* col, const int32_t* col_ptr, const int32_t* eperm, const int32_t* row,
                          float* g_qp, float* g_wk, float* g_hk, float* g_cterm, int N, int H, int D, float scale,
                          void* stream) {
    if (!g || !qp || !wk || !hk || !row_ptr || !col || !col_ptr || !eperm || !row || !g_qp || !g_wk || !g_hk || !g_cterm)
        return fail(SINGA_E_NULL, "edge_logits_bwd: null pointer");
    if (H != 4 || D != 32) return fail(SINGA_E_SHAPE, "edge_logits: built for H = 4 heads, D = 32 key channels per head");
    if (N <= 0) return SINGA_OK;
    hipLaunchKernelGGL((edge_logits_bwd_row_kernel<32, 4>), dim3(kn_grid(N)), dim3(64), 0, (hipStream_t)stream, g,
                       qp, wk, hk, row_ptr, col, g_qp, g_wk, g_cterm, N, scale);
    hipLaunchKernelGGL((edge_logits_bwd_col_kernel<32, 4>), dim3(kn_grid(N)), dim3(64), 0, (hipStream_t)stream, g,
                       qp, wk, col_ptr, eperm, row, g_hk, N, scale);
    return check_launch("edge_logits_bwd");
}

int singa_gather_wsum_fwd(const float* alpha, const float* wv, const float* hv, const int32_t* row_ptr, const int32_t* col,
                          float* out, int N, int H, int F, void* stream) {
    if (!alpha || !wv || !hv || !row_ptr || !col || !out) return fail(SINGA_E_NULL, "gather_wsum_fwd: null pointer");
    if (H != 4 || F != 64) return fail(SINGA_E_SHAPE, "gather_wsum: built for H = 4 heads, F = 64 value channels per head");
    if (N <= 0) return SINGA_OK;
    hipLaunchKernelGGL((gather_wsum_fwd_kernel<4>), dim3(kn_grid(N)), dim3(64), 0, (hipStream_t)stream, alpha, wv,
                       hv, row_ptr, col, out, N);
    return check_launch("gather_wsum_fwd");
}

int singa_gather_wsum_bwd(const float* g, const float* alpha, const float* wv, const float* hv, const int32_t* row_ptr,
                          const int32_t* col, const int32_t* col_ptr, const int32_t* eperm, const int32_t* row,
                          float* g_alpha, float* g_wv, float* g_hv, int N, int H, int F, void* stream) {
    if (!g || !alpha || !wv || !hv || !row_ptr || !col || !col_ptr || !eperm || !row || !g_alpha || !g_wv || !g_hv)
        return fail(SINGA_E_NULL, "gather_wsum_bwd: null pointer");
    if (H != 4 || F != 64) return fail(SINGA_E_SHAPE, "gather_wsum: built for H = 4 heads, F = 64 value channels per head");
    if (N <= 0) return SINGA_OK;
    hipLaunchKernelGGL((gather_wsum_bwd_row_kernel<4>), dim3(kn_grid(N)), dim3(64), 0, (hipStream_t)stream, g,
                       alpha, wv, hv, row_ptr, col, g_alpha, g_wv, N);
    hipLaunchKernelGGL((gather_wsum_bwd_col_kernel<4>), dim3(kn_grid(N)), dim3(64), 0, (hipStream_t)stream, g,
                       alpha, wv, col_ptr, eperm, row, g_hv, N);
    return check_launch("gather_wsum_bwd");
}

#define SINGA_DISPATCH_S2SEP(lmax, edge, ...)                                                            \
    do {                                                                                                 \
        if (edge) {                                                                                      \
            constexpr bool EDGE_ = true; constexpr int C_ = 128;                                         \
            switch (lmax) {                                                                              \
                case 2: { constexpr int L_ = 2; __VA_ARGS__; } break;                                    \
                case 4: { constexpr int L_ = 4; __VA_ARGS__; } break;                                    \
                case 6: { constexpr int L_ = 6; __VA_ARGS__; } break;                                    \
                default: return fail(SINGA_E_LMAX, "s2act_sep: lmax must be 2, 4 or 6");                 \
            }                                                                                            \
        } else {                                                                                         \
            constexpr bool EDGE_ = false; constexpr int C_ = 512;                                        \
            switch (lmax) {                                                                              \
                case 2: { constexpr int L_ = 2; __VA_ARGS__; } break;                                    \
                case 4: { constexpr int L_ = 4; __VA_ARGS__; } break;                                    \
                case 6: { constexpr int L_ = 6; __VA_ARGS__; } break;                                    \
                default: return fail(SINGA_E_LMAX, "s2act_sep: lmax must be 2, 4 or 6");                 \
            }                                                                                            \
        }                                                                                                \
    } while (0)

int singa_s2act_sep_fwd(const singa_seg_t* x, int nseg, const float* gate, int64_t ldg, const float* P, const float* Q,
                        const float* A, float* out, int E, int C, int lmax, void* stream) {
    Segs s;
    if (!pack(x, nseg, &s) || !gate || !P || !Q || !A || !out) return fail(SINGA_E_NULL, "s2act_sep_fwd: null pointer");
    const bool edge = nseg == 3;
    if (!(edge && C == 128) && !(nseg == 1 && C == 512))
        return fail(SINGA_E_SHAPE, "s2act_sep: built for (3 segments, C = 128) and (1 segment, C = 512)");
    if (edge && (s.rows[0] != lmax + 1 || s.rows[1] != 2 * lmax || s.rows[2] != 2 * (lmax - 1)))
        return fail(SINGA_E_SHAPE, "s2act_sep(edge): segment rows must be L+1, 2L, 2(L-1)");
    if (!edge && s.rows[0] != (lmax + 1) * (lmax + 1)) return fail(SINGA_E_SHAPE, "s2act_sep(node): rows must be (L+1)^2");
    if (E <= 0) return SINGA_OK;
    long long EC = (long long)E * C;
    int blocks = (int)((EC + 255) / 256);
    const int tag = edge ? SINGA_PROF_S2_EDGE_FWD : SINGA_PROF_S2_NODE_FWD;
    bool pair = (((uintptr_t)gate | (uintptr_t)out) & 7) == 0 && ldg % 2 == 0 && (edge || lmax <= 4);
    for (int i = 0; i < nseg; ++i) pair = pair && ((uintptr_t)s.p[i] & 7) == 0 && s.ld[i] % 2 == 0;
    if (pair) {
        const long long EC2 = EC / 2;
        blocks = (int)((EC2 + 255) / 256);
        SINGA_DISPATCH_S2SEP(lmax, edge, SINGA_LAUNCH(tag, E, 0, (s2act_sep_fwd2_kernel<L_, EDGE_, C_>), dim3(blocks), dim3(256),
                                                      (hipStream_t)stream, s, gate, (long long)ldg, P, Q, out, EC2));
        return check_launch("s2act_sep_fwd");
    }
    SINGA_DISPATCH_S2SEP(lmax, edge, SINGA_LAUNCH(tag, E, 0, (s2act_sep_fwd_kernel<L_, EDGE_, C_>), dim3(blocks), dim3(256),
                                                  (hipStream_t)stream, s, gate, (long long)ldg, P, Q, A, out, EC));
    return check_launch("s2act_sep_fwd");
}

int singa_s2act_sep_bwd_seg(const singa_seg_t* x, int nseg, const float* gate, int64_t ldg, const float* P, const float* Q,
                            const float* A, const float* g_out, const singa_seg_mut_t* gx, float* g_gate, int64_t ld_gg, int E,
                            int C, int lmax, void* stream) {
    Segs s;
    SegsMut so;
    if (!pack(x, nseg, &s) || !pack_mut(gx, nseg, &so) || !gate || !P || !Q || !A || !g_out || !g_gate)
        return fail(SINGA_E_NULL, "s2act_sep_bwd: null pointer");
    const bool edge = nseg == 3;
    if (!(edge && C == 128) && !(nseg == 1 && C == 512))
        return fail(SINGA_E_SHAPE, "s2act_sep: built for (3 segments, C = 128) and (1 segment, C = 512)");
    if (edge && (s.rows[0] != lmax + 1 || s.rows[1] != 2 * lmax || s.rows[2] != 2 * (lmax - 1)))
        return fail(SINGA_E_SHAPE, "s2act_sep(edge): segment rows must be L+1, 2L, 2(L-1)");
    if (!edge && s.rows[0] != (lmax + 1) * (lmax + 1)) return fail(SINGA_E_SHAPE, "s2act_sep(node): rows must be (L+1)^2");
    for (int i = 0; i < nseg; ++i)
        if (so.rows[i] != s.rows[i] || so.ld[i] < (long long)s.rows[i] * C)
            return fail(SINGA_E_SHAPE, "s2act_sep_bwd: gradient segments must mirror the input segments");
    if (ld_gg < C) return fail(SINGA_E_SHAPE, "s2act_sep_bwd: row stride of g_gate below C");
    if (E <= 0) return SINGA_OK;
    long long EC = (long long)E * C;
    int blocks = (int)((EC + 255) / 256);
    const int tag = edge ? SINGA_PROF_S2_EDGE_BWD : SINGA_PROF_S2_NODE_BWD;
    SINGA_DISPATCH_S2SEP(lmax, edge, SINGA_LAUNCH(tag, E, 0, (s2act_sep_bwd_kernel<L_, EDGE_, C_>), dim3(blocks), dim3(256),
                                                  (hipStream_t)stream, s, gate, (long long)ldg, P, Q, A, g_out, so, g_gate,
                                                  (long long)ld_gg, EC, (const float*)nullptr));
    return check_launch("s2act_sep_bwd");
}

int singa_s2act_ffn_bwd(const float* x, const float* gate, int64_t ldg, const float* P, const float* Q, const float* g_small,
                        const float* W2, float* gx, float* g_gate, int N, int C, int lmax, void* stream) {
    if (!x || !gate || !P || !Q || !g_small || !W2 || !gx || !g_gate) return fail(SINGA_E_NULL, "s2act_ffn_bwd: null pointer");
    if (C != 512) return fail(SINGA_E_SHAPE, "s2act_ffn_bwd: built for the feed-forward block's 512 hidden channels");
    if (ldg < C) return fail(SINGA_E_SHAPE, "s2act_ffn_bwd: row stride of the gate below C");
    if (((uintptr_t)g_small & 15)) return fail(SINGA_E_SHAPE, "s2act_ffn_bwd: g_small must be 16-byte aligned");
    if (N <= 0) return SINGA_OK;
    const int K = (lmax + 1) * (lmax + 1);
    Segs s;
    SegsMut so;
    memset(&s, 0, sizeof(s));
    memset(&so, 0, sizeof(so));
    s.p[0] = x; s.ld[0] = (long long)K * C; s.rows[0] = K;
    so.p[0] = gx; so.ld[0] = (long long)K * C; so.rows[0] = K;
    const long long EC = (long long)N * C;
    const int blocks = (int)(EC / 256);
    const bool edge = false;
    SINGA_DISPATCH_S2SEP(lmax, edge, SINGA_LAUNCH(SINGA_PROF_S2_NODE_BWD, N, 0, (s2act_sep_bwd_kernel<L_, false, 512, true>), dim3(blocks),
                                                  dim3(256), (hipStream_t)stream, s, gate, (long long)ldg, P, Q, (const float*)nullptr,
                                                  g_small, so, g_gate, (long long)C, EC, W2));
    (void)edge;
    return check_launch("s2act_ffn_bwd");
}

int singa_s2act_sep_bwd(const singa_seg_t* x, int nseg, const float* gate, int64_t ldg, const float* P, const float* Q,
                        const float* A, const float* g_out, float* gx, float* g_gate, int E, int C, int lmax,
                        void* stream) {
    if (!x || nseg < 1 || nseg > 3 || !gx) return fail(SINGA_E_NULL, "s2act_sep_bwd: null pointer");
    singa_seg_mut_t o[3];
    long long kin = 0, at = 0;
    for (int i = 0; i < nseg; ++i) kin += x[i].rows;
    for (int i = 0; i < nseg; ++i) {
        o[i].ptr = gx + at * C;
        o[i].ld = kin * C;
        o[i].rows = x[i].rows;
        at += x[i].rows;
    }
    return singa_s2act_sep_bwd_seg(x, nseg, gate, ldg, P, Q, A, g_out, o, g_gate, C, E, C, lmax, stream);
}


int singa_so3_skinny_nparts(int N, int lmax, int C) {
    if (N <= 0 || !so3_skinny_channels_ok(C)) return 0;
    const int runs = C == 512 ? so3_skinny_reduce_runs<512>(lmax) : so3_skinny_reduce_runs<112>(lmax);
    const int npb = so3_skinny_npb(N, runs);
    return (N + npb - 1) / npb;
}

#define SINGA_SKINNY_LC(lmax, C, ...)                                                      \
    do {                                                                                   \
        if ((C) == 512) {                                                                  \
            constexpr int C_ = 512;                                                        \
            switch (lmax) {                                                                \
                case 2: { constexpr int L_ = 2; __VA_ARGS__; } break;                      \
                case 4: { constexpr int L_ = 4; __VA_ARGS__; } break;                      \
                case 6: { constexpr int L_ = 6; __VA_ARGS__; } break;                      \
                default: return fail(SINGA_E_LMAX, "so3_skinny: lmax must be 2, 4 or 6");  \
            }                                                                              \
        } else {                                                                           \
            constexpr int C_ = 112;                                                        \
            switch (lmax) {                                                                \
                case 2: { constexpr int L_ = 2; __VA_ARGS__; } break;                      \
                case 4: { constexpr int L_ = 4; __VA_ARGS__; } break;                      \
                case 6: { constexpr int L_ = 6; __VA_ARGS__; } break;                      \
                default: return fail(SINGA_E_LMAX, "so3_skinny: lmax must be 2, 4 or 6");  \
            }                                                                              \
        }                                                                                  \
    } while (0)

static int g_skinny_valu = 0;
int singa_so3_skinny_variant(int valu) {
    g_skinny_valu = valu ? 1 : 0;
    return SINGA_OK;
}

int singa_so3_skinny_expand(const float* small, const float* W, long long w_l, long long w_c, long long w_u, const float* bias,
                            float* big, int N, int C, int lmax, void* stream) {
    if (!small || !W || !big) return fail(SINGA_E_NULL, "so3_skinny_expand: null pointer");
    if (!so3_skinny_channels_ok(C)) return fail(SINGA_E_SHAPE, "so3_skinny: built for 512 and 112 wide channels");
    if (((uintptr_t)small & 15) || ((uintptr_t)big & 15) || (bias && ((uintptr_t)bias & 15)))
        return fail(SINGA_E_SHAPE, "so3_skinny_expand: 16-byte aligned tensors");
    if (N <= 0) return SINGA_OK;
    hipStream_t st = (hipStream_t)stream;
    if (g_skinny_valu) {
        const int npb = so3_skinny_npb(N, 1536);
        SINGA_SKINNY_LC(lmax, C, hipLaunchKernelGGL((so3_skinny_expand_kernel<L_, C_>),
                                                    dim3((unsigned)(SkinnyCfg<C_>::HALVES * ((N + npb - 1) / npb))),
                                                    dim3(SkinnyCfg<C_>::BLOCK), 0, st, small, W, w_l, w_c, w_u, bias, big, N, npb));
    } else {
        const int npb = (so3_skinny_npb(N, 2048) + 15) / 16 * 16;
        SINGA_SKINNY_LC(lmax, C, hipLaunchKernelGGL((so3_skinny_expand_mfma_kernel<L_, C_>),
                                                    dim3((unsigned)(SkinnyCfg<C_>::HALVES * ((N + npb - 1) / npb))),
                                                    dim3(SkinnyCfg<C_>::BLOCK), 0, st, small, W, w_l, w_c, w_u, bias, big, N, npb));
    }
    return check_launch("so3_skinny_expand");
}

int singa_so3_skinny_reduce(const float* small, const float* big, float* part, int N, int C, int lmax, int out_cu, int bias_row,
                            void* stream) {
    if (!small || !big || !part) return fail(SINGA_E_NULL, "so3_skinny_reduce: null pointer");
    if (!so3_skinny_channels_ok(C)) return fail(SINGA_E_SHAPE, "so3_skinny: built for 512 and 112 wide channels");
    if (N <= 0) return SINGA_OK;
    const int runs = C == 512 ? so3_skinny_reduce_runs<512>(lmax) : so3_skinny_reduce_runs<112>(lmax);
    const int npb = so3_skinny_npb(N, runs);
    hipStream_t st = (hipStream_t)stream;
    if (((uintptr_t)small & 15) || ((uintptr_t)big & 15) || ((uintptr_t)part & 15))
        return fail(SINGA_E_SHAPE, "so3_skinny_reduce: 16-byte aligned tensors");
    if (g_skinny_valu)
        SINGA_SKINNY_LC(lmax, C, hipLaunchKernelGGL((so3_skinny_reduce_kernel<L_, C_>),
                                                    dim3((unsigned)(SkinnyCfg<C_>::HALVES * ((N + npb - 1) / npb))),
                                                    dim3(SkinnyCfg<C_>::BLOCK), 0, st, small, big, part, N, npb, out_cu, bias_row));
    else
        SINGA_SKINNY_LC(lmax, C, hipLaunchKernelGGL((so3_skinny_reduce_mfma_kernel<L_, C_>),
                                                    dim3((unsigned)(SkinnyCfg<C_>::HALVES * ((N + npb - 1) / npb))),
                                                    dim3(SkinnyCfg<C_>::BLOCK), 0, st, small, big, part, N, npb, out_cu, bias_row));
    return check_launch("so3_skinny_reduce");
}

int singa_block_weight_fwd(const float* w, float* out, int h, int k, void* stream) {
    if (!w || !out) return fail(SINGA_E_NULL, "block_weight_fwd: null pointer");
    if (h <= 0 || k <= 0) return SINGA_OK;
    const long long n = 4LL * h * k;
    hipLaunchKernelGGL(block_weight_fwd_kernel, dim3((unsigned)((n + 255) / 256)), dim3(256), 0, (hipStream_t)stream, w, out, h, k);
    return check_launch("block_weight_fwd");
}

int singa_block_weight_bwd(const float* g_block, float* g_w, int h, int k, int accumulate, void* stream) {
    if (!g_block || !g_w) return fail(SINGA_E_NULL, "block_weight_bwd: null pointer");
    if (h <= 0 || k <= 0) return SINGA_OK;
    const long long n = 2LL * h * k;
    hipLaunchKernelGGL(block_weight_bwd_kernel, dim3((unsigned)((n + 255) / 256)), dim3(256), 0, (hipStream_t)stream, g_block, g_w, h, k,
                       accumulate);
    return check_launch("block_weight_bwd");
}

int singa_rowdot_nparts(long long M) { return M <= 0 ? 0 : (int)((M + ROWDOT_ROWS - 1) / ROWDOT_ROWS); }

int singa_rowdot_fwd(const float* x, const float* b, float* out, long long M, int D, float scale, void* stream) {
    if (!x || !b || !out) return fail(SINGA_E_NULL, "rowdot_fwd: null pointer");
    if (D != 32) return fail(SINGA_E_SHAPE, "rowdot: built for 32 channels per row");
    if (((uintptr_t)x & 15) || ((uintptr_t)b & 15)) return fail(SINGA_E_SHAPE, "rowdot: 16-byte aligned operands");
    if (M <= 0) return SINGA_OK;
    hipLaunchKernelGGL(rowdot32_fwd_kernel, dim3((unsigned)((M * 8 + 255) / 256)), dim3(256), 0, (hipStream_t)stream, x, b, out, M, scale);
    return check_launch("rowdot_fwd");
}

int singa_rowdot_bwd(const float* g, const float* x, const float* b, float* gx, float* part, long long M, int D, float scale,
                     void* stream) {
    if (!g || !x || !b || !gx || !part) return fail(SINGA_E_NULL, "rowdot_bwd: null pointer");
    if (D != 32) return fail(SINGA_E_SHAPE, "rowdot: built for 32 channels per row");
    if (((uintptr_t)x & 15) || ((uintptr_t)b & 15) || ((uintptr_t)gx & 15)) return fail(SINGA_E_SHAPE, "rowdot: 16-byte aligned operands");
    if (M <= 0) return SINGA_OK;
    hipLaunchKernelGGL(rowdot32_bwd_kernel, dim3((unsigned)singa_rowdot_nparts(M)), dim3(256), 0, (hipStream_t)stream, g, x, b, gx, part, M,
                       scale);
    return check_launch("rowdot_bwd");
}

static int g_lap_fsi_min = 384;
int singa_lap_pe_fsi_min(int n) {
    if (n < 0) return fail(SINGA_E_SHAPE, "lap_pe_fsi_min: >= 0 (a value above 896 switches the sparse route off)");
    g_lap_fsi_min = n;
    return SINGA_OK;
}

int singa_lap_pe_work(int B, int ld) {
#ifdef SINGA_EMUL
    return (B < 0 || ld < 0) ? 0 : B * (3 + 4 * 9) * ld;
#else
    return (B < 0 || ld < 0) ? 0 : B * LAP_WORK_PER_LD * ld;
#endif
}

int singa_lap_pe(double* A, const int32_t* esrc, const int32_t* edst, const int32_t* eptr, const int32_t* nnodes, const int32_t* first,
                 double* work, float* out, int B, int ld, int kout, void* stream) {
    if (!A || !esrc || !edst || !eptr || !nnodes || !first || !work || !out) return fail(SINGA_E_NULL, "lap_pe: null pointer");
    if (kout < 1 || kout > 8) return fail(SINGA_E_SHAPE, "lap_pe: 1..8 eigenvectors");
    if (ld < 1 || ld > 896) return fail(SINGA_E_SHAPE, "lap_pe: graphs of up to 896 atoms (22.5 vectors of LDS per graph)");
    if (B <= 0) return SINGA_OK;
#ifdef SINGA_EMUL
    return fail(SINGA_E_SHAPE, "lap_pe: not part of the emulation build");
#else
    const int sl = ld < 32 ? 32 : ld;
    const size_t lds = (size_t)((4 + 16) * sl + 16 + 8) * sizeof(double) + (size_t)(5 * sl + 4) * sizeof(int);
    hipStream_t st = (hipStream_t)stream;
    hipError_t e;
    if (ld <= 512) {
        e = hipFuncSetAttribute(reinterpret_cast<const void*>(lap_pe_kernel<8>), hipFuncAttributeMaxDynamicSharedMemorySize, (int)lds);
        if (e != hipSuccess) return fail((int)e, "lap_pe: LDS size refused");
        hipLaunchKernelGGL(lap_pe_kernel<8>, dim3(B), dim3(1024), lds, st, A, esrc, edst, eptr, nnodes, first, work, out, ld, kout, g_lap_fsi_min);
    } else {
        e = hipFuncSetAttribute(reinterpret_cast<const void*>(lap_pe_kernel<16>), hipFuncAttributeMaxDynamicSharedMemorySize, (int)lds);
        if (e != hipSuccess) return fail((int)e, "lap_pe: LDS size refused");
        hipLaunchKernelGGL(lap_pe_kernel<16>, dim3(B), dim3(1024), lds, st, A, esrc, edst, eptr, nnodes, first, work, out, ld, kout, g_lap_fsi_min);
    }
    return check_launch("lap_pe");
#endif
}

int singa_adam_step(float* const* p, const float* const* g, float* const* m, float* const* v, const long long* sizes,
                    const int32_t* chunk_tensor, const long long* chunk_off, int nchunks, int chunk, float* step,
                    const float* lr, float beta1, float beta2, float eps, void* stream) {
    if (!p || !g || !m || !v || !sizes || !chunk_tensor || !chunk_off || !step || !lr)
        return fail(SINGA_E_NULL, "adam_step: null pointer");
    if (nchunks <= 0) return SINGA_OK;
    hipLaunchKernelGGL(adam_kernel, dim3(nchunks), dim3(256), 0, (hipStream_t)stream, p, g, m, v, sizes, chunk_tensor,
                       chunk_off, chunk, step, lr, beta1, beta2, eps);
    hipLaunchKernelGGL(adam_advance_kernel, dim3(1), dim3(64), 0, (hipStream_t)stream, step);
    return check_launch("adam_step");
}

int singa_grad_norm(const float* const* g, const long long* sizes, const int32_t* chunk_tensor, const long long* chunk_off,
                    int nchunks, int chunk, float* partial, float* out, void* stream) {
    if (!g || !sizes || !chunk_tensor || !chunk_off || !partial || !out) return fail(SINGA_E_NULL, "grad_norm: null pointer");
    if (nchunks <= 0) return SINGA_OK;
    hipLaunchKernelGGL(grad_sumsq_kernel, dim3(nchunks), dim3(256), 0, (hipStream_t)stream, g, sizes, chunk_tensor,
                       chunk_off, chunk, partial);
    hipLaunchKernelGGL(grad_norm_finish_kernel, dim3(1), dim3(256), 0, (hipStream_t)stream, partial, nchunks, out);
    return check_launch("grad_norm");
}

int singa_gemm_occupancy(int a_r_contig, int b_r_contig, int cfg) {
    int n = -1;
    hipError_t e = hipErrorInvalidValue;
#define SINGA_OCC(ARC, BRC, CFG) e = hipOccupancyMaxActiveBlocksPerMultiprocessor(&n, gemm_f32_kernel<ARC, BRC, CFG>, 256, 0)
#define SINGA_OCC4(ARC, BRC) do { if (cfg == 0) SINGA_OCC(ARC, BRC, 0); else if (cfg == 1) SINGA_OCC(ARC, BRC, 1); else if (cfg == 2) SINGA_OCC(ARC, BRC, 2); else SINGA_OCC(ARC, BRC, 3); } while (0)
    if (a_r_contig && b_r_contig) SINGA_OCC4(true, true);
    else if (a_r_contig) SINGA_OCC4(true, false);
    else SINGA_OCC4(false, false);
#undef SINGA_OCC4
#undef SINGA_OCC
    return e == hipSuccess ? n : -(int)e;
}

static int g_gemm_force_cfg = -1;
int singa_gemm_force_cfg(int cfg) {
    if (cfg < -1 || cfg > 3) return fail(SINGA_E_SHAPE, "gemm_force_cfg: -1 (automatic), 0 (128x128) or 3 (64x64)");
    g_gemm_force_cfg = cfg;
    return SINGA_OK;
}

int singa_gemm_f32(const singa_gemm_t* probs, int n, int a_r_contig, int b_r_contig, int splits, void* stream) {
    if (!probs || n < 1 || n > SINGA_GEMM_MAX) return fail(SINGA_E_SHAPE, "gemm_f32: 1..SINGA_GEMM_MAX problems per launch");
    if (splits < 1) return fail(SINGA_E_SHAPE, "gemm_f32: splits must be >= 1");
    if (!a_r_contig && b_r_contig) return fail(SINGA_E_SHAPE, "gemm_f32: A output-contiguous with B reduction-contiguous is not built");
    GemmBatch gb;
    memset(&gb, 0, sizeof(gb));
    gb.n = n;
    gb.splits = splits;
    long long rmax = 0;
    int jmax = 0;
    for (int k = 0; k < n; ++k) jmax = probs[k].J > jmax ? probs[k].J : jmax;
    int imax = 0;
    for (int k = 0; k < n; ++k) imax = probs[k].I > imax ? probs[k].I : imax;
    int cfg = jmax <= 32 ? 1 : (imax <= 32 ? 2 : 0);
    if (cfg == 0) {
        long long t128 = 0;
        for (int k = 0; k < n; ++k) t128 += (long long)((probs[k].I + 127) / 128) * ((probs[k].J + 127) / 128);
        if (t128 * splits < 384 || (imax <= 64 && jmax <= 64)) cfg = 3;
        if (g_gemm_force_cfg == 0 || g_gemm_force_cfg == 3) cfg = g_gemm_force_cfg;
    }
    const int BM = cfg == 2 ? 32 : (cfg == 3 ? 64 : 128), BN = cfg == 1 ? 32 : (cfg == 3 ? 64 : 128);
    int tj_total = 0, ti_max = 0, tiles_seq = 0;
    bool same_rows = true;
    for (int k = 1; k < n; ++k) same_rows = same_rows && probs[k].I == probs[0].I;
    for (int k = 0; k < n; ++k) {
        const singa_gemm_t& q = probs[k];
        GemmProb& P = gb.p[k];
        if (!q.a || !q.b || !q.c) return fail(SINGA_E_NULL, "gemm_f32: null operand");
        if (q.I < 0 || q.J < 0 || q.R < 0) return fail(SINGA_E_SHAPE, "gemm_f32: negative size");
        const bool a_ok = a_r_contig ? (q.R % 4 == 0) : (q.I % 4 == 0);
        const bool b_ok = b_r_contig ? (q.R % 4 == 0) : (q.J % 4 == 0);
        if (!a_ok || !b_ok || q.lda % 4 || q.ldb % 4 || q.a_group_ld % 4 || q.b_group_ld % 4 || ((uintptr_t)q.a & 15) ||
            ((uintptr_t)q.b & 15))
            return fail(SINGA_E_SHAPE, "gemm_f32: contiguous axes must be multiples of 4 floats and 16-byte aligned");
        if (b_r_contig && q.b_group > 0) return fail(SINGA_E_SHAPE, "gemm_f32: a reduction-contiguous B has plain rows");
        if (q.J % 4 || q.ldc % 4 || q.c_group_ld % 4 || q.c_split_stride % 4 || ((uintptr_t)q.c & 15) ||
            (q.bias && ((uintptr_t)q.bias & 15)))
            return fail(SINGA_E_SHAPE, "gemm_f32: the result's columns, pitches and base must be multiples of 4 floats / 16 bytes");
        if (splits > 1 && (q.c_group > 0 || q.ldc != q.J || q.bias || q.mask || q.addend || q.relu ||
                           q.c_split_stride < (long long)q.I * q.J))
            return fail(SINGA_E_SHAPE, "gemm_f32: split reductions write dense [I, J] partial slabs (c_split_stride apart), no epilogue options");
        if ((q.mask && q.c_group > 0) || ((uintptr_t)q.mask & 15) || ((uintptr_t)q.addend & 15))
            return fail(SINGA_E_SHAPE, "gemm_f32: mask / addend have the result's layout (a mask: plain rows only) and are 16-byte aligned");
        if (q.asum && (a_r_contig || q.a_group > 0 || q.asum_stride < q.I))
            return fail(SINGA_E_SHAPE, "gemm_f32: asum goes with the (0, 0) form, plain A rows, a slab of at least I floats per split");
        P.A = q.a; P.B = q.b; P.C = q.c; P.bias = q.bias; P.mask = q.mask; P.addend = q.addend; P.relu = q.relu;
        P.asum = q.asum; P.asum_stride = q.asum_stride;
        P.lda = q.lda; P.ldb = q.ldb; P.ldc = q.ldc;
        P.a_group = q.a_group > 0 ? q.a_group : (1 << 30);
        P.b_group = q.b_group > 0 ? q.b_group : (1 << 30);
        P.c_group = q.c_group > 0 ? q.c_group : (1 << 30);
        P.a_gld = q.a_group > 0 ? q.a_group_ld : 0;
        P.b_gld = q.b_group > 0 ? q.b_group_ld : 0;
        P.c_gld = q.c_group > 0 ? q.c_group_ld : 0;
        P.c_split = q.c_split_stride;
        P.I = q.I; P.J = q.J; P.R = q.R;
        P.tiles_j = (q.J + BN - 1) / BN;
        P.tile_begin = same_rows ? tj_total : tiles_seq;
        tj_total += P.tiles_j;
        const int ti = (q.I + BM - 1) / BM;
        tiles_seq += ti * P.tiles_j;
        if (ti > ti_max) ti_max = ti;
        if (q.R > rmax) rmax = q.R;
    }
    const int tiles = same_rows ? ti_max * tj_total : tiles_seq;
    if (tiles == 0) return SINGA_OK;
    gb.tiles_total = tiles;
    gb.tj_total = same_rows ? tj_total : 0;
    gb.r_chunk = splits > 1 ? ((rmax + splits - 1) / splits + 31) / 32 * 32 : (rmax > 0 ? rmax : 1);
    const long long nblk = (long long)tiles * splits;
    if (nblk > (1 << 30)) return fail(SINGA_E_SHAPE, "gemm_f32: too many tiles");
    const dim3 grid((unsigned)((nblk + 7) / 8 * 8)), block(256);
    hipStream_t st = (hipStream_t)stream;
#define SINGA_GEMM_GO(tag, ARC, BRC)                                                                        \
    do {                                                                                                    \
        if (cfg == 1) SINGA_LAUNCH(tag, 0, tiles, (gemm_f32_kernel<ARC, BRC, 1>), grid, block, st, gb);     \
        else if (cfg == 2) SINGA_LAUNCH(tag, 0, tiles, (gemm_f32_kernel<ARC, BRC, 2>), grid, block, st, gb); \
        else if (cfg == 3) SINGA_LAUNCH(tag, 0, tiles, (gemm_f32_kernel<ARC, BRC, 3>), grid, block, st, gb); \
        else SINGA_LAUNCH(tag, 0, tiles, (gemm_f32_kernel<ARC, BRC, 0>), grid, block, st, gb);              \
    } while (0)
    if (a_r_contig && b_r_contig) SINGA_GEMM_GO(SINGA_PROF_GEMM_NT, true, true);
    else if (a_r_contig) SINGA_GEMM_GO(SINGA_PROF_GEMM_NN, true, false);
    else SINGA_GEMM_GO(SINGA_PROF_GEMM_TN, false, false);
#undef SINGA_GEMM_GO
    return check_launch("gemm_f32");
}

int singa_cgemm3m_f32(const singa_cgemm_t* probs, int n, int a_r_contig, int b_r_contig, int splits, void* stream) {
    if (!probs || n < 1 || n > SINGA_CGEMM_MAX) return fail(SINGA_E_SHAPE, "cgemm3m_f32: 1..SINGA_CGEMM_MAX problems per launch");
    if (splits < 1) return fail(SINGA_E_SHAPE, "cgemm3m_f32: splits must be >= 1");
    if (!a_r_contig && b_r_contig) return fail(SINGA_E_SHAPE, "cgemm3m_f32: A output-contiguous with B reduction-contiguous is not built");
    CGemmBatch gb;
    memset(&gb, 0, sizeof(gb));
    gb.n = n;
    gb.splits = splits;
    constexpr int BM = 128, BN = 64;
    long long rmax = 0;
    int tj_total = 0, ti_max = 0, tiles_seq = 0;
    bool same_rows = true;
    for (int k = 1; k < n; ++k) same_rows = same_rows && probs[k].I == probs[0].I;
    for (int k = 0; k < n; ++k) {
        const singa_cgemm_t& q = probs[k];
        CGemmProb& P = gb.p[k];
        if (!q.a || !q.b || !q.c) return fail(SINGA_E_NULL, "cgemm3m_f32: null operand");
        if (q.I < 0 || q.J < 0 || q.R < 0) return fail(SINGA_E_SHAPE, "cgemm3m_f32: negative size");
        const bool a_ok = a_r_contig ? (q.R % 4 == 0) : (q.I % 4 == 0);
        const bool b_ok = b_r_contig ? (q.R % 4 == 0) : (q.J % 4 == 0);
        if (!a_ok || !b_ok || q.J % 4 || q.lda % 4 || q.ldb % 4 || q.ldc % 4 || q.a_im % 4 || q.b_im % 4 || q.c_im % 4 ||
            q.c_split_stride % 4 || ((uintptr_t)q.a & 15) || ((uintptr_t)q.b & 15) || ((uintptr_t)q.c & 15))
            return fail(SINGA_E_SHAPE, "cgemm3m_f32: contiguous axes, pitches and part offsets must be multiples of 4 floats, bases 16-byte aligned");
        if (q.sigma != 1.0f && q.sigma != -1.0f) return fail(SINGA_E_SHAPE, "cgemm3m_f32: sigma is +1 or -1");
        if (splits > 1 && q.c_split_stride <= 0) return fail(SINGA_E_SHAPE, "cgemm3m_f32: split reductions need c_split_stride");
        P.A = q.a; P.B = q.b; P.C = q.c;
        P.lda = q.lda; P.ldb = q.ldb; P.ldc = q.ldc;
        P.a_im = q.a_im; P.b_im = q.b_im; P.c_im = q.c_im;
        P.c_split = q.c_split_stride;
        P.I = q.I; P.J = q.J; P.R = q.R;
        P.sigma = q.sigma;
        P.tiles_j = (q.J + BN - 1) / BN;
        P.tile_begin = same_rows ? tj_total : tiles_seq;
        tj_total += P.tiles_j;
        const int ti = (q.I + BM - 1) / BM;
        tiles_seq += ti * P.tiles_j;
        if (ti > ti_max) ti_max = ti;
        if (q.R > rmax) rmax = q.R;
    }
    const int tiles = same_rows ? ti_max * tj_total : tiles_seq;
    if (tiles == 0) return SINGA_OK;
    gb.tiles_total = tiles;
    gb.tj_total = same_rows ? tj_total : 0;
    gb.r_chunk = splits > 1 ? ((rmax + splits - 1) / splits + 15) / 16 * 16 : (rmax > 0 ? rmax : 1);
    const long long nblk = (long long)tiles * splits;
    if (nblk > (1 << 30)) return fail(SINGA_E_SHAPE, "cgemm3m_f32: too many tiles");
    const dim3 grid((unsigned)((nblk + 7) / 8 * 8)), block(256);
    hipStream_t st = (hipStream_t)stream;
    if (a_r_contig && b_r_contig) SINGA_LAUNCH(SINGA_PROF_CGEMM_NT, 0, tiles, (cgemm3m_f32_kernel<true, true>), grid, block, st, gb);
    else if (a_r_contig) SINGA_LAUNCH(SINGA_PROF_CGEMM_NN, 0, tiles, (cgemm3m_f32_kernel<true, false>), grid, block, st, gb);
    else SINGA_LAUNCH(SINGA_PROF_CGEMM_TN, 0, tiles, (cgemm3m_f32_kernel<false, false>), grid, block, st, gb);
    return check_launch("cgemm3m_f32");
}

int singa_alpha_logits_nslots(int E) {
    long long slots = ((long long)E + 0) < 1 ? 1 : E;
    long long cap = 256 * 8 * 8;
    return (int)(slots < cap ? ((slots + 7) / 8) * 8 : cap);
}

int singa_alpha_logits_fwd(const float* h0, long long ld, const float* ln_w, const float* ln_b, const float* dot, float* logits,
                           int E, int heads, int A, float eps, void* stream) {
    if (!h0 || !ln_w || !ln_b || !dot || !logits) return fail(SINGA_E_NULL, "alpha_logits_fwd: null pointer");
    if (heads != 7 || A != 32) return fail(SINGA_E_SHAPE, "alpha_logits: built for 7 heads x 32 alpha channels");
    if (E <= 0) return SINGA_OK;
    int blocks = singa_alpha_logits_nslots(E) / 8;
    hipLaunchKernelGGL((alpha_logits_fwd_kernel<7>), dim3(blocks), dim3(256), 0, (hipStream_t)stream, h0, ld, ln_w, ln_b, dot,
                       logits, E, eps);
    return check_launch("alpha_logits_fwd");
}

int singa_alpha_logits_bwd_ld(const float* h0, long long ld, const float* ln_w, const float* ln_b, const float* dot,
                              const float* g_logits, float* g_x, long long ld_gx, float* part, int E, int heads, int A, float eps,
                              void* stream) {
    if (!h0 || !ln_w || !ln_b || !dot || !g_logits || !g_x || !part) return fail(SINGA_E_NULL, "alpha_logits_bwd: null pointer");
    if (heads != 7 || A != 32) return fail(SINGA_E_SHAPE, "alpha_logits: built for 7 heads x 32 alpha channels");
    if (ld_gx < (long long)heads * A) return fail(SINGA_E_SHAPE, "alpha_logits_bwd: row stride of g_x below heads * A");
    if (E <= 0) return SINGA_OK;
    int blocks = singa_alpha_logits_nslots(E) / 8;
    hipLaunchKernelGGL((alpha_logits_bwd_kernel<7>), dim3(blocks), dim3(256), 0, (hipStream_t)stream, h0, ld, ln_w, ln_b, dot,
                       g_logits, g_x, ld_gx, part, E, eps);
    return check_launch("alpha_logits_bwd");
}

int singa_alpha_logits_bwd(const float* h0, long long ld, const float* ln_w, const float* ln_b, const float* dot,
                           const float* g_logits, float* g_x, float* part, int E, int heads, int A, float eps, void* stream) {
    return singa_alpha_logits_bwd_ld(h0, ld, ln_w, ln_b, dot, g_logits, g_x, (long long)heads * A, part, E, heads, A, eps, stream);
}

int singa_ln_silu_nparts(long long M) {
    long long blocks = (M + 63) / 64;
    return (int)(blocks < 256 ? (blocks < 1 ? 1 : blocks) : 256) * 64;
}

int singa_ln_silu_fwd(const float* x, const float* gamma, const float* beta, float* out, long long M, int C, float eps,
                      void* stream) {
    if (!x || !gamma || !beta || !out) return fail(SINGA_E_NULL, "ln_silu_fwd: null pointer");
    if (C != 16) return fail(SINGA_E_SHAPE, "ln_silu: built for rows of 16 channels");
    if (M <= 0) return SINGA_OK;
    long long blocks = (M + 63) / 64;
    hipLaunchKernelGGL((ln_silu_fwd_kernel<16>), dim3((unsigned)(blocks < 4096 ? blocks : 4096)), dim3(64), 0,
                       (hipStream_t)stream, x, gamma, beta, out, M, eps);
    return check_launch("ln_silu_fwd");
}

int singa_ln_silu_bwd(const float* x, const float* gamma, const float* beta, const float* g_out, float* g_x, float* part,
                      long long M, int C, float eps, void* stream) {
    if (!x || !gamma || !beta || !g_out || !g_x || !part) return fail(SINGA_E_NULL, "ln_silu_bwd: null pointer");
    if (C != 16) return fail(SINGA_E_SHAPE, "ln_silu: built for rows of 16 channels");
    if (M <= 0) return SINGA_OK;
    hipLaunchKernelGGL((ln_silu_bwd_kernel<16>), dim3(singa_ln_silu_nparts(M) / 64), dim3(64), 0, (hipStream_t)stream, x, gamma,
                       beta, g_out, g_x, part, M, eps);
    return check_launch("ln_silu_bwd");
}

int singa_bias_ssp_fwd(const float* u, const float* b, float* y, long long M, int n, void* stream) {
    if (!u || !b || !y) return fail(SINGA_E_NULL, "bias_ssp_fwd: null pointer");
    if (n <= 0 || n % 4) return fail(SINGA_E_SHAPE, "bias_ssp: row length must be a positive multiple of 4");
    if (M <= 0) return SINGA_OK;
    const long long total4 = M * n / 4;
    hipLaunchKernelGGL(bias_ssp_fwd_kernel, dim3((unsigned)((total4 + 255) / 256)), dim3(256), 0, (hipStream_t)stream, u, b, y,
                       total4, n);
    return check_launch("bias_ssp_fwd");
}

int singa_bias_ssp_bwd(const float* u, const float* b, const float* g, float* gu, long long M, int n, void* stream) {
    if (!u || !b || !g || !gu) return fail(SINGA_E_NULL, "bias_ssp_bwd: null pointer");
    if (n <= 0 || n % 4) return fail(SINGA_E_SHAPE, "bias_ssp: row length must be a positive multiple of 4");
    if (M <= 0) return SINGA_OK;
    const long long total4 = M * n / 4;
    hipLaunchKernelGGL(bias_ssp_bwd_kernel, dim3((unsigned)((total4 + 255) / 256)), dim3(256), 0, (hipStream_t)stream, u, b, g, gu,
                       total4, n);
    return check_launch("bias_ssp_bwd");
}

int singa_ln256_nparts(long long M) {
    long long blocks = (M + 3) / 4;
    return (int)(blocks < 1 ? 1 : (blocks < 1024 ? blocks : 1024)) * 4;
}

int singa_ln256_fwd(const float* a, const float* r, const float* gamma, const float* beta, float* y, long long M, int C,
                    float eps, void* stream) {
    if (!a || !gamma || !beta || !y) return fail(SINGA_E_NULL, "ln256_fwd: null pointer");
    if (C != 256) return fail(SINGA_E_SHAPE, "ln256: built for rows of 256 channels");
    if (M <= 0) return SINGA_OK;
    long long blocks = (M + 3) / 4;
    hipLaunchKernelGGL(ln256_fwd_kernel, dim3((unsigned)(blocks < 8192 ? blocks : 8192)), dim3(256), 0, (hipStream_t)stream, a, r,
                       gamma, beta, y, M, eps);
    return check_launch("ln256_fwd");
}

int singa_ln256_bwd(const float* a, const float* r, const float* gamma, const float* g, float* gs, float* part, long long M,
                    int C, float eps, void* stream) {
    if (!a || !gamma || !g || !gs || !part) return fail(SINGA_E_NULL, "ln256_bwd: null pointer");
    if (C != 256) return fail(SINGA_E_SHAPE, "ln256: built for rows of 256 channels");
    if (M <= 0) return SINGA_OK;
    hipLaunchKernelGGL(ln256_bwd_kernel, dim3(singa_ln256_nparts(M) / 4), dim3(256), 0, (hipStream_t)stream, a, r, gamma, g, gs,
                       part, M, eps);
    return check_launch("ln256_bwd");
}

int singa_dec_self_attn(const float* x, const float* wqkv_t, const float* bqkv, const float* wo_t, const float* bo,
                        const float* gamma, const float* beta, float* k_cache, float* v_cache, const long long* pos, int R, int P,
                        float* y, float eps, void* stream) {
    if (!x || !wqkv_t || !bqkv || !wo_t || !bo || !gamma || !beta || !k_cache || !v_cache || !pos || !y)
        return fail(SINGA_E_NULL, "dec_self_attn: null pointer");
    if (P <= 0 || P > 256) return fail(SINGA_E_SHAPE, "dec_self_attn: built for at most 256 cached positions");
    if (R <= 0) return SINGA_OK;
    hipLaunchKernelGGL(dec_self_attn_kernel, dim3(R), dim3(1024), 0, (hipStream_t)stream, x, wqkv_t, bqkv, wo_t, bo, gamma, beta,
                       k_cache, v_cache, pos, P, y, eps);
    return check_launch("dec_self_attn");
}

int singa_dec_cross_attn(const float* y, const float* wq_t, const float* bq, const float* ck, const float* cv,
                         const unsigned char* pad, const float* wo_t, const float* bo, const float* gamma, const float* beta,
                         int R, int beams, int S, float* z, float eps, void* stream) {
    if (!y || !wq_t || !bq || !ck || !cv || !pad || !wo_t || !bo || !gamma || !beta || !z)
        return fail(SINGA_E_NULL, "dec_cross_attn: null pointer");
    if (S <= 0 || S > DEC_MAX_S) return fail(SINGA_E_SHAPE, "dec_cross_attn: built for at most 1024 encoder positions");
    if (beams <= 0 || R % beams) return fail(SINGA_E_SHAPE, "dec_cross_attn: rows must be proteins x beams");
    if (R <= 0) return SINGA_OK;
    hipLaunchKernelGGL(dec_cross_attn_kernel, dim3(R), dim3(1024), 0, (hipStream_t)stream, y, wq_t, bq, ck, cv, pad, wo_t, bo, gamma,
                       beta, beams, S, z, eps);
    return check_launch("dec_cross_attn");
}

int singa_dec_ffn(const float* z, const float* w1_t, const float* b1, const float* w2_t, const float* b2, const float* gamma,
                  const float* beta, int R, float* out, float eps, void* stream) {
    if (!z || !w1_t || !b1 || !w2_t || !b2 || !gamma || !beta || !out) return fail(SINGA_E_NULL, "dec_ffn: null pointer");
    if (R <= 0) return SINGA_OK;
    hipLaunchKernelGGL(dec_ffn_kernel, dim3(R), dim3(1024), 0, (hipStream_t)stream, z, w1_t, b1, w2_t, b2, gamma, beta, out, eps);
    return check_launch("dec_ffn");
}

int singa_sample_token(const float* logits, const float* uniforms, const unsigned char* allowed, const long long* pos,
                       int pos_offset, int rows, int V, int T, float tau, int top_k, float top_p, int eos, int pad,
                       unsigned char* finished, int32_t* length, float* sum_logp, long long* tokens, long long* next,
                       int32_t* live, float* tok_logp, void* stream) {
    if (!logits || !uniforms || !pos || !finished || !length || !sum_logp || !tokens || !next || !live)
        return fail(SINGA_E_NULL, "sample_token: null pointer");
    if (V < 1 || V > 1024) return fail(SINGA_E_SHAPE, "sample_token: vocabulary of 1..1024 tokens");
    if (!(tau >= 0.f)) return fail(SINGA_E_SHAPE, "sample_token: temperature must be >= 0");
    if (top_k < 0) return fail(SINGA_E_SHAPE, "sample_token: top_k must be >= 0 (0 = off)");
    if (!(top_p > 0.f && top_p <= 1.f)) return fail(SINGA_E_SHAPE, "sample_token: top_p must be in (0, 1]");
    if (T < 2 || eos < 0 || eos >= V || pad < 0 || pad >= V || rows < 0)
        return fail(SINGA_E_SHAPE, "sample_token: T >= 2 columns, eos / pad inside the vocabulary");
    if (rows == 0) return SINGA_OK;
#ifdef SINGA_EMUL
    return fail(SINGA_E_SHAPE, "sample_token: not part of the emulation build");
#else
    const dim3 grid((rows + 3) / 4), block(256);
    hipStream_t st = (hipStream_t)stream;
#define SINGA_SAMPLE_LAUNCH(NPL)                                                                                              \
    hipLaunchKernelGGL((sample_token_kernel<NPL, false, false>), grid, block, 0, st, logits, uniforms, allowed, pos, pos_offset, rows, V, \
                       T, tau, top_k, top_p, eos, pad, finished, length, sum_logp, tokens, next, live, tok_logp,                  \
                       (const unsigned char*)nullptr, (int32_t*)nullptr, (float*)nullptr, (const long long*)nullptr,                  \
                       (int32_t*)nullptr)
    if (V <= 128) SINGA_SAMPLE_LAUNCH(2);
    else if (V <= 256) SINGA_SAMPLE_LAUNCH(4);
    else if (V <= 512) SINGA_SAMPLE_LAUNCH(8);
    else SINGA_SAMPLE_LAUNCH(16);
#undef SINGA_SAMPLE_LAUNCH
    return check_launch("sample_token");
#endif
}

int singa_sample_token_grammar(const float* logits, const float* uniforms, const unsigned char* allowed,
                               const unsigned char* cls, const long long* pos, int pos_offset, int rows, int V, int T, float tau,
                               int top_k, float top_p, int eos, int pad, unsigned char* finished, int32_t* length,
                               float* sum_logp, long long* tokens, long long* next, int32_t* live, float* tok_logp,
                               int32_t* gstate, float* allowed_logp, void* stream) {
    if (!logits || !uniforms || !pos || !finished || !length || !sum_logp || !tokens || !next || !live || !cls || !gstate)
        return fail(SINGA_E_NULL, "sample_token_grammar: null pointer");
    if (V < 1 || V > 1024) return fail(SINGA_E_SHAPE, "sample_token_grammar: vocabulary of 1..1024 tokens");
    if (!(tau >= 0.f)) return fail(SINGA_E_SHAPE, "sample_token_grammar: temperature must be >= 0");
    if (top_k < 0) return fail(SINGA_E_SHAPE, "sample_token_grammar: top_k must be >= 0 (0 = off)");
    if (!(top_p > 0.f && top_p <= 1.f)) return fail(SINGA_E_SHAPE, "sample_token_grammar: top_p must be in (0, 1]");
    if (T < 3 || eos < 0 || eos >= V || pad < 0 || pad >= V || rows < 0)
        return fail(SINGA_E_SHAPE, "sample_token_grammar: T >= 3 columns, eos / pad inside the vocabulary");
    if (rows == 0) return SINGA_OK;
#ifdef SINGA_EMUL
    return fail(SINGA_E_SHAPE, "sample_token_grammar: not part of the emulation build");
#else
    const dim3 grid((rows + 3) / 4), block(256);
    hipStream_t st = (hipStream_t)stream;
#define SINGA_SAMPLE_LAUNCH(NPL)                                                                                              \
    hipLaunchKernelGGL((sample_token_kernel<NPL, true, false>), grid, block, 0, st, logits, uniforms, allowed, pos, pos_offset, rows, V, \
                       T, tau, top_k, top_p, eos, pad, finished, length, sum_logp, tokens, next, live, tok_logp, cls, gstate,     \
                       allowed_logp, (const long long*)nullptr, (int32_t*)nullptr)
    if (V <= 128) SINGA_SAMPLE_LAUNCH(2);
    else if (V <= 256) SINGA_SAMPLE_LAUNCH(4);
    else if (V <= 512) SINGA_SAMPLE_LAUNCH(8);
    else SINGA_SAMPLE_LAUNCH(16);
#undef SINGA_SAMPLE_LAUNCH
    return check_launch("sample_token_grammar");
#endif
}

int singa_sample_token_forced(const float* logits, const float* uniforms, const unsigned char* allowed,
                              const unsigned char* cls, const long long* pos, int pos_offset, int rows, int V, int T, float tau,
                              int top_k, float top_p, int eos, int pad, unsigned char* finished, int32_t* length,
                              float* sum_logp, long long* tokens, long long* next, int32_t* live, float* tok_logp,
                              int32_t* gstate, float* allowed_logp, const long long* forced, int32_t* rank, void* stream) {
    const bool grammar = cls && gstate;
    if (!logits || !uniforms || !pos || !finished || !length || !sum_logp || !tokens || !next || !live || !forced)
        return fail(SINGA_E_NULL, "sample_token_forced: null pointer");
    if (!grammar && (cls || gstate || allowed_logp))
        return fail(SINGA_E_NULL, "sample_token_forced: cls and gstate go together (allowed_logp only with them)");
    if (V < 1 || V > 1024) return fail(SINGA_E_SHAPE, "sample_token_forced: vocabulary of 1..1024 tokens");
    if (!(tau >= 0.f)) return fail(SINGA_E_SHAPE, "sample_token_forced: temperature must be >= 0");
    if (top_k < 0) return fail(SINGA_E_SHAPE, "sample_token_forced: top_k must be >= 0 (0 = off)");
    if (!(top_p > 0.f && top_p <= 1.f)) return fail(SINGA_E_SHAPE, "sample_token_forced: top_p must be in (0, 1]");
    if (T < (grammar ? 3 : 2) || eos < 0 || eos >= V || pad < 0 || pad >= V || rows < 0)
        return fail(SINGA_E_SHAPE, "sample_token_forced: T >= 2 columns (3 under the grammar), eos / pad inside the vocabulary");
    if (rows == 0) return SINGA_OK;
#ifdef SINGA_EMUL
    return fail(SINGA_E_SHAPE, "sample_token_forced: not part of the emulation build");
#else
    const dim3 grid((rows + 3) / 4), block(256);
    hipStream_t st = (hipStream_t)stream;
#define SINGA_SAMPLE_LAUNCH(NPL)                                                                                              \
    do {                                                                                                                      \
        if (grammar)                                                                                                          \
            hipLaunchKernelGGL((sample_token_kernel<NPL, true, true>), grid, block, 0, st, logits, uniforms, allowed, pos,    \
                               pos_offset, rows, V, T, tau, top_k, top_p, eos, pad, finished, length, sum_logp, tokens, next, \
                               live, tok_logp, cls, gstate, allowed_logp, forced, rank);                                      \
        else                                                                                                                  \
            hipLaunchKernelGGL((sample_token_kernel<NPL, false, true>), grid, block, 0, st, logits, uniforms, allowed, pos,   \
                               pos_offset, rows, V, T, tau, top_k, top_p, eos, pad, finished, length, sum_logp, tokens, next, \
                               live, tok_logp, cls, gstate, allowed_logp, forced, rank);                                      \
    } while (0)
    if (V <= 128) SINGA_SAMPLE_LAUNCH(2);
    else if (V <= 256) SINGA_SAMPLE_LAUNCH(4);
    else if (V <= 512) SINGA_SAMPLE_LAUNCH(8);
    else SINGA_SAMPLE_LAUNCH(16);
#undef SINGA_SAMPLE_LAUNCH
    return check_launch("sample_token_forced");
#endif
}

int singa_smiles_rule_host(const unsigned char* cls, const int32_t* state, const int32_t* rem, int n, unsigned char* ok,
                           int32_t* next_state) {
    if (!cls || !state || !rem || !ok || !next_state) return fail(SINGA_E_NULL, "smiles_rule_host: null pointer");
    if (n < 0) return fail(SINGA_E_SHAPE, "smiles_rule_host: n must be >= 0");
    for (int i = 0; i < n; ++i) {
        ok[i] = smiles_allows(state[i], cls[i], rem[i]) ? 1 : 0;
        next_state[i] = ok[i] ? smiles_next(state[i], cls[i]) : state[i];
    }
    return SINGA_OK;
}

int singa_edge_mlp_fwd(const float* attr, const float* w1tk, const float* b1k, const float* w2tk, const float* b2k,
                       const float* w1tv, const float* b1v, const float* w2tv, const float* b2v, float* wk, float* wv, int E,
                       int CIN, int HK, int HV, void* stream) {
    if (!attr || !w1tk || !b1k || !w2tk || !b2k || !w1tv || !b1v || !w2tv || !b2v || !wk || !wv)
        return fail(SINGA_E_NULL, "edge_mlp_fwd: null pointer");
    if (CIN != 64 || HK != 32 || HV != 64)
        return fail(SINGA_E_SHAPE, "edge_mlp: built for 64 edge channels, 32 key / 64 value channels per head");
    if (E <= 0) return SINGA_OK;
    const long long tiles = ((long long)E + 31) / 32;
    const long long blocks = (tiles + 3) / 4;
    hipLaunchKernelGGL(edge_mlp_mfma_fwd_kernel, dim3((unsigned)(blocks < 768 ? blocks : 768)), dim3(256), 0, (hipStream_t)stream,
                       attr, w1tk, b1k, w2tk, b2k, w1tv, b1v, w2tv, b2v, wk, wv, E);
    return check_launch("edge_mlp_fwd");
}

int singa_edge_mlp_bwd_nparts(int E, int H) {
    const long long blocks = (((long long)E + 31) / 32 + 3) / 4;
    const long long cap = H <= 32 ? 512 : 256;
    return (int)(blocks < cap ? (blocks < 1 ? 1 : blocks) : cap);
}

int singa_edge_mlp_bwd(const float* attr, const float* g_out, const float* w1t, const float* b1, const float* w2, float* part,
                       int E, int CIN, int H, void* stream) {
    if (!attr || !g_out || !w1t || !b1 || !w2 || !part) return fail(SINGA_E_NULL, "edge_mlp_bwd: null pointer");
    if (CIN != 64 || (H != 32 && H != 64))
        return fail(SINGA_E_SHAPE, "edge_mlp: built for 64 edge channels, 32 key / 64 value channels per head");
    if (E <= 0) return SINGA_OK;
    const int blocks = singa_edge_mlp_bwd_nparts(E, H);
    if (H == 32)
        hipLaunchKernelGGL((edge_mlp_mfma_bwd_kernel<32>), dim3(blocks, 1), dim3(256), 0, (hipStream_t)stream, attr, g_out, w1t,
                           b1, w2, part, E);
    else
        hipLaunchKernelGGL((edge_mlp_mfma_bwd_kernel<64>), dim3(blocks, 2), dim3(256), 0, (hipStream_t)stream, attr, g_out, w1t,
                           b1, w2, part, E);
    return check_launch("edge_mlp_bwd");
}

int singa_masked_softmax_fwd(const float* s, const unsigned char* mask, long long mask_stride_b, long long mask_stride_t, float* p,
                             int BH, int T, int S, int heads, float scale, void* stream) {
// ... 190 lines not shown
```

Measured before the change: 865.4.

## Make GEMM and CGEMM kernels persistent with next-tile prefetch during epilogue

Turns the f32 GEMM and complex 3M GEMM kernels into persistent kernels. The grid is capped at the occupancy-derived number of resident workgroups, and each workgroup loops over tiles, keeping the XCD-strided assignment. While it writes one tile's epilogue, it decodes the next tile and issues that tile's first global loads, and problem parameters are read straight from the kernarg segment. This aims to cut launch/tail overhead and hide the prologue load latency, at the cost of more register pressure, more complex control flow, and possible load imbalance when the tile count is small.

```diff
diff --git a/singa_amd/csrc/singa_hip.hip b/singa_amd/csrc/singa_hip.hip
--- a/singa_amd/csrc/singa_hip.hip
+++ b/singa_amd/csrc/singa_hip.hip
@@ -3533,6 +3533,13 @@
     }
 }
 
+#ifndef SINGA_EMUL
+#define SINGA_KARG_AS __attribute__((address_space(4)))
+#define SINGA_KARG(T, arg) ((const SINGA_KARG_AS T*)__builtin_amdgcn_kernarg_segment_ptr())
+#else
+#define SINGA_KARG_AS
+#define SINGA_KARG(T, arg) (&(arg))
+#endif
 struct GemmProb {
     const float* A;
     const float* B;
@@ -3573,46 +3580,72 @@
     float* const Bs0 = smem + 2 * SZA;
     const int nblk = gb.tiles_total * gb.splits;
     const int per = (nblk + 7) >> 3;
-    const int id = (int)(blockIdx.x & 7) * per + (int)(blockIdx.x >> 3);
-    if (id >= nblk) return;
-    const int split = id / gb.tiles_total;
-    const int tile = id - split * gb.tiles_total;
-    const int ti = gb.tj_total ? tile / gb.tj_total : 0, trem = gb.tj_total ? tile - ti * gb.tj_total : tile;
-    int pi = 0;
-#pragma unroll
-    for (int q = 1; q < SINGA_GEMM_MAX; ++q)
-        if (q < gb.n && trem >= gb.p[q].tile_begin) pi = q;
-    const GemmProb& P = gb.p[pi];
-    const int local = trem - P.tile_begin;
-    const int i0 = (gb.tj_total ? ti : local / P.tiles_j) * BM, j0 = (gb.tj_total ? local : local % P.tiles_j) * BN;
-    const long long r_begin = (long long)split * gb.r_chunk;
-    const long long r_end = (r_begin + gb.r_chunk < P.R) ? r_begin + gb.r_chunk : P.R;
+    const int xcd = (int)(blockIdx.x & 7), gx = (int)(gridDim.x >> 3);
+    int kk = (int)(blockIdx.x >> 3);
+    if (kk >= per || xcd * per + kk >= nblk) return;
     const int tid = threadIdx.x, lane = tid & 63, wave = tid >> 6;
-    const int wrow = CFG == 0 ? (wave >> 1) * 64 : (CFG == 1 ? wave * 32 : (CFG == 3 ? (wave >> 1) * 32 : 0));
-    const int wcol = CFG == 0 ? (wave & 1) * 64 : (CFG == 1 ? 0 : (CFG == 3 ? (wave & 1) * 32 : wave * 32));
+    auto wrow_of = [](int w) { return CFG == 0 ? (w >> 1) * 64 : (CFG == 1 ? w * 32 : (CFG == 3 ? (w >> 1) * 32 : 0)); };
+    auto wcol_of = [](int w) { return CFG == 0 ? (w & 1) * 64 : (CFG == 1 ? 0 : (CFG == 3 ? (w & 1) * 32 : w * 32)); };
+    const int wrow = wrow_of(wave), wcol = wcol_of(wave);
     const int l31 = lane & 31, half = lane >> 5;
     const int kq = tid & 7, rr = tid >> 3;
 
+    const SINGA_KARG_AS GemmBatch* const kb = SINGA_KARG(GemmBatch, gb);
+    const SINGA_KARG_AS GemmProb* Pp = &kb->p[0];
+    int split = 0, i0 = 0, j0 = 0;
+    long long r_begin = 0, r_end = 0, nsteps = 0;
+    int last8 = 0;
     const float* arow[NA];
     const float* brow[NB];
-    if (A_RC) {
-#pragma unroll
-        for (int j = 0; j < NA; ++j) {
-            const int i = i0 + rr + 32 * j;
-            const long long off = P.a_group == (1 << 30) ? (long long)i * P.lda
-                                                         : (long long)(i / P.a_group) * P.a_gld + (long long)(i % P.a_group) * P.lda;
-            arow[j] = i < P.I ? P.A + off + 4 * kq : nullptr;
-        }
-    }
-    if (B_RC) {
-#pragma unroll
-        for (int j = 0; j < NB; ++j) {
-            const int jj = j0 + rr + 32 * j;
-            brow[j] = jj < P.J ? P.B + (long long)jj * P.ldb + 4 * kq : nullptr;
-        }
-    }
+    bool full = false, allc = false, do_asum = false;
+    unsigned blkv = 0;
+    auto decode = [&](int id, int t) __attribute__((always_inline)) {
+        const int kq = t & 7, rr = t >> 3, wrow = wrow_of(t >> 6), wcol = wcol_of(t >> 6);
+        split = id / gb.tiles_total;
+        const int tile = id - split * gb.tiles_total;
+        const int ti = gb.tj_total ? tile / gb.tj_total : 0, trem = gb.tj_total ? tile - ti * gb.tj_total : tile;
+        int pi = 0;
+#pragma unroll
+        for (int q = 1; q < SINGA_GEMM_MAX; ++q)
+            if (q < gb.n && trem >= gb.p[q].tile_begin) pi = q;
+        Pp = &kb->p[pi];
+        const SINGA_KARG_AS GemmProb& P = *Pp;
+        const int local = trem - P.tile_begin;
+        i0 = (gb.tj_total ? ti : local / P.tiles_j) * BM;
+        j0 = (gb.tj_total ? local : local % P.tiles_j) * BN;
+        r_begin = (long long)split * gb.r_chunk;
+        r_end = (r_begin + gb.r_chunk < P.R) ? r_begin + gb.r_chunk : P.R;
+        if (A_RC) {
+#pragma unroll
+            for (int j = 0; j < NA; ++j) {
+                const int i = i0 + rr + 32 * j;
+                const long long off = P.a_group == (1 << 30) ? (long long)i * P.lda
+                                                             : (long long)(i / P.a_group) * P.a_gld + (long long)(i % P.a_group) * P.lda;
+                arow[j] = i < P.I ? P.A + off + 4 * kq : nullptr;
+            }
+        }
+        if (B_RC) {
+#pragma unroll
+            for (int j = 0; j < NB; ++j) {
+                const int jj = j0 + rr + 32 * j;
+                brow[j] = jj < P.J ? P.B + (long long)jj * P.ldb + 4 * kq : nullptr;
+            }
+        }
+        full = i0 + BM <= P.I && j0 + BN <= P.J && r_end > r_begin && (r_end - r_begin) % BK == 0;
+        allc = full && P.a_group == (1 << 30) && P.b_group == (1 << 30);
+        do_asum = !A_RC && P.asum != nullptr && j0 == 0;
+        nsteps = r_end > r_begin ? (r_end - r_begin + BK - 1) / BK : 0;
+        last8 = nsteps > 0 ? (int)((r_end - r_begin - (nsteps - 1) * BK + 7) / 8) : 0;
+        unsigned bv = 0;
+#pragma unroll
+        for (int a = 0; a < MT; ++a)
+#pragma unroll
+            for (int b = 0; b < NT; ++b)
+                bv |= ((i0 + wrow + 32 * a < P.I) && (j0 + wcol + 32 * b < P.J) ? 1u : 0u) << (a * NT + b);
+        blkv = __builtin_amdgcn_readfirstlane(bv);
+    };
     float4 ra0[NA], rb0[NB], ra1[NA], rb1[NB];
-    const bool full = i0 + BM <= P.I && j0 + BN <= P.J && r_end > r_begin && (r_end - r_begin) % BK == 0;
+    unsigned ma0 = 0, mb0 = 0, ma1 = 0, mb1 = 0;
     auto load_rc = [&](auto all_c, float4* reg, unsigned& mask, const float* const* rows, const float* dummy, int n, long long r0) {
         if constexpr (decltype(all_c)::value) {
 #pragma unroll
@@ -3665,13 +3698,32 @@
             *reinterpret_cast<float4*>(S + (rq + rows * j) * pitch + 4 * c4) = (mask >> j) & 1u ? reg[j] : make_float4(0.f, 0.f, 0.f, 0.f);
     };
     auto load_ab = [&](auto all_c, float4* ra, float4* rb, unsigned& ma, unsigned& mb, long long r0) __attribute__((always_inline)) {
+        const SINGA_KARG_AS GemmProb& P = *Pp;
         if (A_RC) load_rc(all_c, ra, ma, arow, P.A, NA, r0);
         else load_oc(all_c, ra, ma, P.A, P.lda, P.a_group, P.a_gld, i0, P.I, NA, BM / 4, r0);
         if (B_RC) load_rc(all_c, rb, mb, brow, P.B, NB, r0);
         else load_oc(all_c, rb, mb, P.B, P.ldb, P.b_group, P.b_gld, j0, P.J, NB, BN / 4, r0);
     };
-    const bool do_asum = !A_RC && P.asum != nullptr && j0 == 0;
-    const float asum_on = do_asum ? 1.f : 0.f;
+    auto load_first = [&](auto all_c) __attribute__((always_inline)) {
+        const float4 z4 = make_float4(0.f, 0.f, 0.f, 0.f);
+        if (nsteps > 0) load_ab(all_c, ra0, rb0, ma0, mb0, r_begin);
+        else {
+#pragma unroll
+            for (int j = 0; j < NA; ++j) ra0[j] = z4;
+#pragma unroll
+            for (int j = 0; j < NB; ++j) rb0[j] = z4;
+            ma0 = mb0 = 0;
+        }
+        if (nsteps > 1) load_ab(all_c, ra1, rb1, ma1, mb1, r_begin + BK);
+        else {
+#pragma unroll
+            for (int j = 0; j < NA; ++j) ra1[j] = z4;
+#pragma unroll
+            for (int j = 0; j < NB; ++j) rb1[j] = z4;
+            ma1 = mb1 = 0;
+        }
+    };
+    float asum_on = 0.f;
     float4 asum4 = make_float4(0.f, 0.f, 0.f, 0.f);
     auto store_ab = [&](const float4* ra, const float4* rb, unsigned ma, unsigned mb, int buf) __attribute__((always_inline)) {
         if constexpr (!A_RC) {
@@ -3699,20 +3751,7 @@
     };
 
     floatx16 acc[MT][NT];
-#pragma unroll
-    for (int a = 0; a < MT; ++a)
-#pragma unroll
-        for (int b = 0; b < NT; ++b)
-#pragma unroll
-            for (int r = 0; r < 16; ++r) acc[a][b][r] = 0.f;
-
-    unsigned blkv = 0;
-#pragma unroll
-    for (int a = 0; a < MT; ++a)
-#pragma unroll
-        for (int b = 0; b < NT; ++b)
-            blkv |= ((i0 + wrow + 32 * a < P.I) && (j0 + wcol + 32 * b < P.J) ? 1u : 0u) << (a * NT + b);
-    blkv = __builtin_amdgcn_readfirstlane(blkv);
+
     auto compute = [&](auto edge_c, int buf, int nt8) __attribute__((always_inline)) {
         const float* Sa = As0 + buf * SZA;
         const float* Sb = Bs0 + buf * SZB;
@@ -3747,8 +3786,6 @@
         }
     };
 
-    const long long nsteps = r_end > r_begin ? (r_end - r_begin + BK - 1) / BK : 0;
-    const int last8 = nsteps > 0 ? (int)((r_end - r_begin - (nsteps - 1) * BK + 7) / 8) : 0;
     auto pipeline = [&](auto interior_c) __attribute__((always_inline)) {
 #if SINGA_GEMM_PIPE
         if constexpr (CFG == 0 && decltype(interior_c)::value) {
@@ -3778,13 +3815,6 @@
     };
     auto k_loop = [&](auto all_c) __attribute__((always_inline)) {
         constexpr std::integral_constant<bool, !decltype(all_c)::value> edge_c{};
-        unsigned ma0 = 0, mb0 = 0, ma1 = 0, mb1 = 0;
-        if (nsteps > 0) {
-            load_ab(all_c, ra0, rb0, ma0, mb0, r_begin);
-            if (nsteps > 1) load_ab(all_c, ra1, rb1, ma1, mb1, r_begin + BK);
-            store_ab(ra0, rb0, ma0, mb0, 0);
-        }
-        __syncthreads();
         long long st = 0;
 #if !defined(SINGA_GEMM_LAB_NOLOAD) && !defined(SINGA_GEMM_LAB_NOSYNC)
         if (nsteps > 3) __builtin_amdgcn_s_waitcnt(0x0F70);
@@ -3831,57 +3861,105 @@
 #endif
         }
     };
-    if (full && P.a_group == (1 << 30) && P.b_group == (1 << 30)) k_loop(std::true_type{});
-    else k_loop(std::false_type{});
-    if (!A_RC && do_asum) {
-        constexpr int W4 = BM / 4, RG = 256 / W4;
-        float* red = smem;
-        *reinterpret_cast<float4*>(red + (tid / W4) * BM + 4 * (tid % W4)) = asum4;
-        __syncthreads();
-        if (tid < BM) {
-            float t = 0.f;
-#pragma unroll
-            for (int g2 = 0; g2 < RG; ++g2) t += red[g2 * BM + tid];
-            if (i0 + tid < P.I) P.asum[(long long)split * P.asum_stride + i0 + tid] = t;
-        }
-        __syncthreads();
-    }
-    float* Cb = P.C + (long long)split * P.c_split;
-    float* stage = smem + wave * (32 * PE);
     constexpr int C4 = 8 * NT;
     constexpr int ROWS_PER_PASS = 64 / C4, PASSES = 32 / ROWS_PER_PASS;
-    const int c4 = lane % C4, rsub = lane / C4;
-    const int jcol = j0 + wcol + 4 * c4;
-    float4 bias4 = make_float4(0.f, 0.f, 0.f, 0.f);
-    if (P.bias && jcol < P.J) bias4 = *reinterpret_cast<const float4*>(P.bias + jcol);
-#pragma unroll
-    for (int a = 0; a < MT; ++a) {
-        __builtin_amdgcn_wave_barrier();
-#pragma unroll
-        for (int b = 0; b < NT; ++b)
-#pragma unroll
-            for (int q = 0; q < 16; ++q) stage[((q & 3) + 8 * (q >> 2) + 4 * half) * PE + 32 * b + l31] = acc[a][b][q];
-        __builtin_amdgcn_wave_barrier();
-#pragma unroll
-        for (int ps = 0; ps < PASSES; ++ps) {
-            const int rloc = rsub + ROWS_PER_PASS * ps;
-            const int i = i0 + wrow + 32 * a + rloc;
-            float4 v = *reinterpret_cast<const float4*>(stage + rloc * PE + 4 * c4);
-            if (i < P.I && jcol < P.J) {
-                v.x += bias4.x; v.y += bias4.y; v.z += bias4.z; v.w += bias4.w;
-                const long long row = P.c_group == (1 << 30) ? (long long)i * P.ldc
-                                                             : (long long)(i / P.c_group) * P.c_gld + (long long)(i % P.c_group) * P.ldc;
-                if (P.addend) {
-                    const float4 ad = *reinterpret_cast<const float4*>(P.addend + row + jcol);
-                    v.x += ad.x; v.y += ad.y; v.z += ad.z; v.w += ad.w;
+
+    constexpr bool AHEAD = A_RC && (CFG == 0 || CFG == 3);
+    auto run = [&](auto all_c) __attribute__((always_inline)) {
+      load_first(all_c);
+      for (;;) {
+        asum_on = do_asum ? 1.f : 0.f;
+        asum4 = make_float4(0.f, 0.f, 0.f, 0.f);
+#pragma unroll
+        for (int a = 0; a < MT; ++a)
+#pragma unroll
+            for (int b = 0; b < NT; ++b)
+#pragma unroll
+                for (int r = 0; r < 16; ++r) acc[a][b][r] = 0.f;
+        if (nsteps > 0) store_ab(ra0, rb0, ma0, mb0, 0);
+        __syncthreads();
+        k_loop(all_c);
+
+        int te = threadIdx.x;
+        SINGA_KEEP_VGPR(te);
+        const int tid = te, lane = tid & 63, wave = tid >> 6, wrow = wrow_of(wave), wcol = wcol_of(wave);
+        const int l31 = lane & 31, half = lane >> 5;
+        float* stage = smem + wave * (32 * PE);
+        const int c4 = lane % C4, rsub = lane / C4;
+        const SINGA_KARG_AS GemmProb& P = *Pp;
+        const int ei0 = i0, ej0 = j0, esplit = split;
+        const bool e_asum = do_asum;
+        const int jcol = ej0 + wcol + 4 * c4;
+        auto crow = [&](int i) __attribute__((always_inline)) {
+            return P.c_group == (1 << 30) ? (long long)i * P.ldc
+                                          : (long long)(i / P.c_group) * P.c_gld + (long long)(i % P.c_group) * P.ldc;
+        };
+        kk += gx;
+        const bool more = kk < per && xcd * per + kk < nblk;
+        float4 bias4 = make_float4(0.f, 0.f, 0.f, 0.f);
+        if (P.bias && jcol < P.J) bias4 = *reinterpret_cast<const float4*>(P.bias + jcol);
+        bool same = false;
+        if (more) {
+            decode(xcd * per + kk, tid);
+            same = allc == decltype(all_c)::value;
+            if (AHEAD && same) load_first(all_c);
+        }
+        __builtin_amdgcn_sched_barrier(0);
+        if (!A_RC && e_asum) {
+            constexpr int W4 = BM / 4, RG = 256 / W4;
+            float* red = smem;
+            *reinterpret_cast<float4*>(red + (tid / W4) * BM + 4 * (tid % W4)) = asum4;
+            __syncthreads();
+            if (tid < BM) {
+                float t = 0.f;
+#pragma unroll
+                for (int g2 = 0; g2 < RG; ++g2) t += red[g2 * BM + tid];
+                if (ei0 + tid < P.I) P.asum[(long long)esplit * P.asum_stride + ei0 + tid] = t;
+            }
+            __syncthreads();
+        }
+        float* Cb = P.C + (long long)esplit * P.c_split;
+#pragma unroll
+        for (int a = 0; a < MT; ++a) {
+            __builtin_amdgcn_wave_barrier();
+#pragma unroll
+            for (int b = 0; b < NT; ++b)
+#pragma unroll
+                for (int q = 0; q < 16; ++q) stage[((q & 3) + 8 * (q >> 2) + 4 * half) * PE + 32 * b + l31] = acc[a][b][q];
+            __builtin_amdgcn_wave_barrier();
+#pragma unroll
+            for (int ps = 0; ps < PASSES; ++ps) {
+                const int rloc = rsub + ROWS_PER_PASS * ps;
+                const int i = ei0 + wrow + 32 * a + rloc;
+                float4 v = *reinterpret_cast<const float4*>(stage + rloc * PE + 4 * c4);
+                if (i < P.I && jcol < P.J) {
+                    v.x += bias4.x; v.y += bias4.y; v.z += bias4.z; v.w += bias4.w;
+                    const long long row = crow(i);
+                    if (P.addend) {
+                        const float4 ad = *reinterpret_cast<const float4*>(P.addend + row + jcol);
+                        v.x += ad.x; v.y += ad.y; v.z += ad.z; v.w += ad.w;
+                    }
+                    if (P.relu) { v.x = fmaxf(v.x, 0.f); v.y = fmaxf(v.y, 0.f); v.z = fmaxf(v.z, 0.f); v.w = fmaxf(v.w, 0.f); }
+                    if (P.mask) {
+                        const float4 m = *reinterpret_cast<const float4*>(P.mask + row + jcol);
+                        v.x = m.x > 0.f ? v.x : 0.f; v.y = m.y > 0.f ? v.y : 0.f; v.z = m.z > 0.f ? v.z : 0.f; v.w = m.w > 0.f ? v.w : 0.f;
+                    }
+                    *reinterpret_cast<float4*>(Cb + row + jcol) = v;
                 }
-                if (P.relu) { v.x = fmaxf(v.x, 0.f); v.y = fmaxf(v.y, 0.f); v.z = fmaxf(v.z, 0.f); v.w = fmaxf(v.w, 0.f); }
-                if (P.mask) {
-                    const float4 m = *reinterpret_cast<const float4*>(P.mask + row + jcol);
-                    v.x = m.x > 0.f ? v.x : 0.f; v.y = m.y > 0.f ? v.y : 0.f; v.z = m.z > 0.f ? v.z : 0.f; v.w = m.w > 0.f ? v.w : 0.f;
-                }
-                *reinterpret_cast<float4*>(Cb + row + jcol) = v;
-            }
+            }
+        }
+        if (!more) return true;
+        if (!AHEAD && same) load_first(all_c);
+        __syncthreads();
+        if (!same) return false;
+      }
+    };
+    decode(xcd * per + kk, tid);
+    for (;;) {
+        if (allc) {
+            if (run(std::true_type{})) break;
+        } else {
+            if (run(std::false_type{})) break;
         }
     }
 }
@@ -3921,44 +3999,61 @@
     float* const Bs0 = smem + 2 * SZA;
     const int nblk = gb.tiles_total * gb.splits;
     const int per = (nblk + 7) >> 3;
-    const int id = (int)(blockIdx.x & 7) * per + (int)(blockIdx.x >> 3);
-    if (id >= nblk) return;
-    const int split = id / gb.tiles_total;
-    const int tile = id - split * gb.tiles_total;
-    const int ti = gb.tj_total ? tile / gb.tj_total : 0, trem = gb.tj_total ? tile - ti * gb.tj_total : tile;
-    int pi = 0;
-#pragma unroll
-    for (int q = 1; q < SINGA_CGEMM_MAX; ++q)
-        if (q < gb.n && trem >= gb.p[q].tile_begin) pi = q;
-    const CGemmProb& P = gb.p[pi];
-    const int local = trem - P.tile_begin;
-    const int i0 = (gb.tj_total ? ti : local / P.tiles_j) * BM, j0 = (gb.tj_total ? local : local % P.tiles_j) * BN;
-    const long long r_begin = (long long)split * gb.r_chunk;
-    const long long r_end = (r_begin + gb.r_chunk < P.R) ? r_begin + gb.r_chunk : P.R;
+    const int xcd = (int)(blockIdx.x & 7), gx = (int)(gridDim.x >> 3);
+    int kk = (int)(blockIdx.x >> 3);
+    if (kk >= per || xcd * per + kk >= nblk) return;
     const int tid = threadIdx.x, lane = tid & 63, wave = tid >> 6;
     const int wrow = (wave >> 1) * 64, wcol = (wave & 1) * 32;
     const int l31 = lane & 31, half = lane >> 5;
-    const float sigma = P.sigma;
 
     const int kq = tid & 3, pt = (tid >> 2) & 1, rr = tid >> 3;
+    const SINGA_KARG_AS CGemmBatch* const kb = SINGA_KARG(CGemmBatch, gb);
+    const SINGA_KARG_AS CGemmProb* Pp = &kb->p[0];
+    int split = 0, i0 = 0, j0 = 0;
+    long long r_begin = 0, r_end = 0, nsteps = 0;
+    float sigma = 1.f;
     const float* arow[NA];
     const float* brow[NB];
-    if (A_RC) {
-#pragma unroll
-        for (int j = 0; j < NA; ++j) {
-            const int i = i0 + rr + 32 * j;
-            arow[j] = i < P.I ? P.A + (long long)i * P.lda + (long long)pt * P.a_im + 4 * kq : nullptr;
-        }
-    }
-    if (B_RC) {
-#pragma unroll
-        for (int j = 0; j < NB; ++j) {
-            const int jj = j0 + rr + 32 * j;
-            brow[j] = jj < P.J ? P.B + (long long)jj * P.ldb + (long long)pt * P.b_im + 4 * kq : nullptr;
-        }
-    }
+    bool full = false;
+    bool row1 = false, colv = false;
+    auto decode = [&](int id, int t) __attribute__((always_inline)) {
+        const int kq = t & 3, pt = (t >> 2) & 1, rr = t >> 3, wrow = (t >> 7) * 64, wcol = ((t >> 6) & 1) * 32;
+        split = id / gb.tiles_total;
+        const int tile = id - split * gb.tiles_total;
+        const int ti = gb.tj_total ? tile / gb.tj_total : 0, trem = gb.tj_total ? tile - ti * gb.tj_total : tile;
+        int pi = 0;
+#pragma unroll
+        for (int q = 1; q < SINGA_CGEMM_MAX; ++q)
+            if (q < gb.n && trem >= gb.p[q].tile_begin) pi = q;
+        Pp = &kb->p[pi];
+        const SINGA_KARG_AS CGemmProb& P = *Pp;
+        const int local = trem - P.tile_begin;
+        i0 = (gb.tj_total ? ti : local / P.tiles_j) * BM;
+        j0 = (gb.tj_total ? local : local % P.tiles_j) * BN;
+        r_begin = (long long)split * gb.r_chunk;
+        r_end = (r_begin + gb.r_chunk < P.R) ? r_begin + gb.r_chunk : P.R;
+        sigma = P.sigma;
+        if (A_RC) {
+#pragma unroll
+            for (int j = 0; j < NA; ++j) {
+                const int i = i0 + rr + 32 * j;
+                arow[j] = i < P.I ? P.A + (long long)i * P.lda + (long long)pt * P.a_im + 4 * kq : nullptr;
+            }
+        }
+        if (B_RC) {
+#pragma unroll
+            for (int j = 0; j < NB; ++j) {
+                const int jj = j0 + rr + 32 * j;
+                brow[j] = jj < P.J ? P.B + (long long)jj * P.ldb + (long long)pt * P.b_im + 4 * kq : nullptr;
+            }
+        }
+        full = i0 + BM <= P.I && j0 + BN <= P.J && r_end > r_begin && (r_end - r_begin) % BK == 0;
+        nsteps = r_end > r_begin ? (r_end - r_begin + BK - 1) / BK : 0;
+        row1 = __builtin_amdgcn_readfirstlane((int)(i0 + wrow + 32 < P.I)) != 0;
+        colv = __builtin_amdgcn_readfirstlane((int)(j0 + wcol < P.J)) != 0;
+    };
     float4 ra0[NA], rb0[NB], ra1[NA], rb1[NB];
-    const bool full = i0 + BM <= P.I && j0 + BN <= P.J && r_end > r_begin && (r_end - r_begin) % BK == 0;
+    unsigned ma0 = 0, mb0 = 0, ma1 = 0, mb1 = 0;
     auto load_rc = [&](auto all_c, float4* reg, unsigned& mask, const float* const* rows, const float* dummy, int n, long long r0) {
         if constexpr (decltype(all_c)::value) {
 #pragma unroll
@@ -4018,10 +4113,30 @@
         }
     };
     auto load_ab = [&](auto all_c, float4* ra, float4* rb, unsigned& ma, unsigned& mb, long long r0) __attribute__((always_inline)) {
+        const SINGA_KARG_AS CGemmProb& P = *Pp;
         if (A_RC) load_rc(all_c, ra, ma, arow, P.A, NA, r0);
         else load_oc(all_c, ra, ma, P.A, P.lda, P.a_im, i0, P.I, NA, BM / 4, r0);
         if (B_RC) load_rc(all_c, rb, mb, brow, P.B, NB, r0);
         else load_oc(all_c, rb, mb, P.B, P.ldb, P.b_im, j0, P.J, NB, BN / 4, r0);
+    };
+    auto load_first = [&](auto all_c) __attribute__((always_inline)) {
+        const float4 z4 = make_float4(0.f, 0.f, 0.f, 0.f);
+        if (nsteps > 0) load_ab(all_c, ra0, rb0, ma0, mb0, r_begin);
+        else {
+#pragma unroll
+            for (int j = 0; j < NA; ++j) ra0[j] = z4;
+#pragma unroll
+            for (int j = 0; j < NB; ++j) rb0[j] = z4;
+            ma0 = mb0 = 0;
+        }
+        if (nsteps > 1) load_ab(all_c, ra1, rb1, ma1, mb1, r_begin + BK);
+        else {
+#pragma unroll
+            for (int j = 0; j < NA; ++j) ra1[j] = z4;
+#pragma unroll
+            for (int j = 0; j < NB; ++j) rb1[j] = z4;
+            ma1 = mb1 = 0;
+        }
     };
     auto store_ab = [&](const float4* ra, const float4* rb, unsigned ma, unsigned mb, int buf) __attribute__((always_inline)) {
         if (A_RC) store_rc(As0 + buf * SZA, SZA1, ra, ma, NA);
@@ -4040,12 +4155,6 @@
         }
     };
     floatx16 acc1[2], acc2[2], acc3[2];
-#pragma unroll
-    for (int a = 0; a < 2; ++a)
-#pragma unroll
-        for (int r = 0; r < 16; ++r) acc1[a][r] = acc2[a][r] = acc3[a][r] = 0.f;
-    const bool row1 = __builtin_amdgcn_readfirstlane((int)(i0 + wrow + 32 < P.I)) != 0;
-    const bool colv = __builtin_amdgcn_readfirstlane((int)(j0 + wcol < P.J)) != 0;
     auto compute = [&](auto all_c, int buf) __attribute__((always_inline)) {
         if constexpr (!decltype(all_c)::value) {
             if (!colv) return;
@@ -4077,7 +4186,6 @@
             }
         }
     };
-    const long long nsteps = r_end > r_begin ? (r_end - r_begin + BK - 1) / BK : 0;
     auto pipeline = [&](auto interior_c) __attribute__((always_inline)) {
 #if SINGA_CGEMM_PIPE
         if constexpr (decltype(interior_c)::value) {
@@ -4099,13 +4207,6 @@
 #endif
     };
     auto k_loop = [&](auto all_c) __attribute__((always_inline)) {
-        unsigned ma0 = 0, mb0 = 0, ma1 = 0, mb1 = 0;
-        if (nsteps > 0) {
-            load_ab(all_c, ra0, rb0, ma0, mb0, r_begin);
-            if (nsteps > 1) load_ab(all_c, ra1, rb1, ma1, mb1, r_begin + BK);
-            store_ab(ra0, rb0, ma0, mb0, 0);
-        }
-        __syncthreads();
         long long st = 0;
         if (nsteps > 3) __builtin_amdgcn_s_waitcnt(0x0F70);
         for (; st + 3 < nsteps; st += 2) {
@@ -4136,29 +4237,67 @@
             __syncthreads();
         }
     };
-    if (full) k_loop(std::true_type{});
-    else k_loop(std::false_type{});
-    float* Cb = P.C + (long long)split * P.c_split;
-    float* stage = smem + wave * (32 * PE);
-    const int c4 = lane & 15, rsub = lane >> 4;
-    const int part = c4 >> 3, jcol = j0 + wcol + 4 * (c4 & 7);
-#pragma unroll
-    for (int a = 0; a < 2; ++a) {
-        __builtin_amdgcn_wave_barrier();
-#pragma unroll
-        for (int q = 0; q < 16; ++q) {
-            const int rw = (q & 3) + 8 * (q >> 2) + 4 * half;
-            stage[rw * PE + l31] = acc1[a][q] - acc3[a][q];
-            stage[rw * PE + 32 + l31] = acc1[a][q] + acc2[a][q];
-        }
-        __builtin_amdgcn_wave_barrier();
-#pragma unroll
-        for (int ps = 0; ps < 8; ++ps) {
-            const int rloc = rsub + 4 * ps;
-            const int i = i0 + wrow + 32 * a + rloc;
-            const float4 v = *reinterpret_cast<const float4*>(stage + rloc * PE + 4 * c4);
-            if (i < P.I && jcol < P.J)
-                *reinterpret_cast<float4*>(Cb + (long long)i * P.ldc + (long long)part * P.c_im + jcol) = v;
+
+    auto run = [&](auto all_c) __attribute__((always_inline)) {
+      load_first(all_c);
+      for (;;) {
+#pragma unroll
+        for (int a = 0; a < 2; ++a)
+#pragma unroll
+            for (int r = 0; r < 16; ++r) acc1[a][r] = acc2[a][r] = acc3[a][r] = 0.f;
+        if (nsteps > 0) store_ab(ra0, rb0, ma0, mb0, 0);
+        __syncthreads();
+        k_loop(all_c);
+        int te = threadIdx.x;
+        SINGA_KEEP_VGPR(te);
+        const int tid = te, lane = tid & 63, wave = tid >> 6, wrow = (wave >> 1) * 64, wcol = (wave & 1) * 32;
+        const int l31 = lane & 31, half = lane >> 5;
+        float* stage = smem + wave * (32 * PE);
+        const int c4 = lane & 15, rsub = lane >> 4;
+        const int part = c4 >> 3;
+        const SINGA_KARG_AS CGemmProb& P = *Pp;
+        const int ei0 = i0, esplit = split;
+        const int jcol = j0 + wcol + 4 * (c4 & 7);
+        kk += gx;
+        const bool more = kk < per && xcd * per + kk < nblk;
+        bool same = false;
+        if (more) {
+            decode(xcd * per + kk, tid);
+            same = full == decltype(all_c)::value;
+            if (same) load_first(all_c);
+        }
+        __builtin_amdgcn_sched_barrier(0);
+        float* Cb = P.C + (long long)esplit * P.c_split;
+#pragma unroll
+        for (int a = 0; a < 2; ++a) {
+            __builtin_amdgcn_wave_barrier();
+#pragma unroll
+            for (int q = 0; q < 16; ++q) {
+                const int rw = (q & 3) + 8 * (q >> 2) + 4 * half;
+                stage[rw * PE + l31] = acc1[a][q] - acc3[a][q];
+                stage[rw * PE + 32 + l31] = acc1[a][q] + acc2[a][q];
+            }
+            __builtin_amdgcn_wave_barrier();
+#pragma unroll
+            for (int ps = 0; ps < 8; ++ps) {
+                const int rloc = rsub + 4 * ps;
+                const int i = ei0 + wrow + 32 * a + rloc;
+                const float4 v = *reinterpret_cast<const float4*>(stage + rloc * PE + 4 * c4);
+                if (i < P.I && jcol < P.J)
+                    *reinterpret_cast<float4*>(Cb + (long long)i * P.ldc + (long long)part * P.c_im + jcol) = v;
+            }
+        }
+        if (!more) return true;
+        __syncthreads();
+        if (!same) return false;
+      }
+    };
+    decode(xcd * per + kk, tid);
+    for (;;) {
+        if (full) {
+            if (run(std::true_type{})) break;
+        } else {
+            if (run(std::false_type{})) break;
         }
     }
 }
@@ -5200,6 +5339,7 @@
 
 const char* singa_last_error_string(void) { return g_err; }
 
+static void gemm_slots_fill();
 int singa_init(const double* jd_flat, int lmax_max) {
     if (!jd_flat) return fail(SINGA_E_NULL, "singa_init: jd_flat is null");
     if (lmax_max < 0 || lmax_max > 11) return fail(SINGA_E_LMAX, "singa_init: lmax_max must be in [0, 11]");
@@ -5212,6 +5352,7 @@
         return (int)e;
     }
     g_lmax_init = lmax_max;
+    gemm_slots_fill();
     return SINGA_OK;
 }
 
@@ -5815,6 +5956,40 @@
 #undef SINGA_OCC4
 #undef SINGA_OCC
     return e == hipSuccess ? n : -(int)e;
+}
+
+static int g_gemm_slots[3][4], g_cgemm_slots[3];
+static int g_gemm_max_wg = 0;
+static bool g_gemm_slots_filled = false;
+static void gemm_slots_fill() {
+    if (g_gemm_slots_filled) return;
+    g_gemm_slots_filled = true;
+    int dev = 0, cus = 0;
+    hipDeviceProp_t prop;
+    if (hipGetDevice(&dev) == hipSuccess && hipGetDeviceProperties(&prop, dev) == hipSuccess) cus = prop.multiProcessorCount;
+    auto slots = [&](int occ) { return occ > 0 && cus > 0 ? occ * cus / 8 * 8 : 0; };
+    for (int f = 0; f < 3; ++f) {
+        for (int c = 0; c < 4; ++c) g_gemm_slots[f][c] = c == 1 || c == 2 ? 0 : slots(singa_gemm_occupancy(f < 2, f == 0, c));
+        int n = 0;
+        hipError_t e;
+        if (f == 0) e = hipOccupancyMaxActiveBlocksPerMultiprocessor(&n, cgemm3m_f32_kernel<true, true>, 256, 0);
+        else if (f == 1) e = hipOccupancyMaxActiveBlocksPerMultiprocessor(&n, cgemm3m_f32_kernel<true, false>, 256, 0);
+        else e = hipOccupancyMaxActiveBlocksPerMultiprocessor(&n, cgemm3m_f32_kernel<false, false>, 256, 0);
+        g_cgemm_slots[f] = e == hipSuccess ? slots(n) : 0;
+    }
+}
+static unsigned gemm_grid(long long nblk, int slots) {
+    static bool env_read = false;
+    if (!env_read) {
+        env_read = true;
+        const char* env = getenv("SINGA_GEMM_MAX_WG");
+        const int v = env && *env ? atoi(env) : 0;
+        if (v >= 8) g_gemm_max_wg = v / 8 * 8;
+    }
+    long long g = (nblk + 7) / 8 * 8;
+    if (slots > 0 && g > slots) g = slots;
+    if (g_gemm_max_wg > 0 && g > g_gemm_max_wg) g = g_gemm_max_wg;
+    return (unsigned)g;
 }
 
 static int g_gemm_force_cfg = -1;
@@ -5895,7 +6070,8 @@
     gb.r_chunk = splits > 1 ? ((rmax + splits - 1) / splits + 31) / 32 * 32 : (rmax > 0 ? rmax : 1);
     const long long nblk = (long long)tiles * splits;
     if (nblk > (1 << 30)) return fail(SINGA_E_SHAPE, "gemm_f32: too many tiles");
-    const dim3 grid((unsigned)((nblk + 7) / 8 * 8)), block(256);
+    gemm_slots_fill();
+    const dim3 grid(gemm_grid(nblk, g_gemm_slots[a_r_contig ? (b_r_contig ? 0 : 1) : 2][cfg])), block(256);
     hipStream_t st = (hipStream_t)stream;
 #define SINGA_GEMM_GO(tag, ARC, BRC)                                                                        \
     do {                                                                                                    \
@@ -5957,7 +6133,8 @@
     gb.r_chunk = splits > 1 ? ((rmax + splits - 1) / splits + 15) / 16 * 16 : (rmax > 0 ? rmax : 1);
     const long long nblk = (long long)tiles * splits;
     if (nblk > (1 << 30)) return fail(SINGA_E_SHAPE, "cgemm3m_f32: too many tiles");
-    const dim3 grid((unsigned)((nblk + 7) / 8 * 8)), block(256);
+    gemm_slots_fill();
+    const dim3 grid(gemm_grid(nblk, g_cgemm_slots[a_r_contig ? (b_r_contig ? 0 : 1) : 2])), block(256);
     hipStream_t st = (hipStream_t)stream;
     if (a_r_contig && b_r_contig) SINGA_LAUNCH(SINGA_PROF_CGEMM_NT, 0, tiles, (cgemm3m_f32_kernel<true, true>), grid, block, st, gb);
     else if (a_r_contig) SINGA_LAUNCH(SINGA_PROF_CGEMM_NN, 0, tiles, (cgemm3m_f32_kernel<true, false>), grid, block, st, gb);
```

Result: slower. 852.1 (-1.5%).
